# kkty/kmer-sets-compression

Hardware: AMD Instinct MI355X
Metric: Mk-mers/s processed in kmerset-multiple-compress; bytes/k-mer after SPSS (higher is better)
Workload: dtype u32

## Files before the change

### kmer-sets-compression_amd/csrc/ksh_encode.hip

```cpp
#include "ksh_internal.h"
#include "ksh_dsu.h"
#include "ksh_kmer.h"

#include <algorithm>
#include <cstddef>
#include <cstdlib>
#include <string>

namespace ksh {

#ifndef KSH_RULER_SHIFT
#define KSH_RULER_SHIFT 5
#endif
constexpr int kRulerShift = KSH_RULER_SHIFT;
constexpr uint32_t kRulerEvery = 1u << kRulerShift;

constexpr uint32_t kNone = 0xFFFFFFFFu;
constexpr uint32_t kMulti = 0xFFFFFFFEu;

#ifndef KSH_JUMP_HOPS
#define KSH_JUMP_HOPS 4
#endif
constexpr int kJumpHops = KSH_JUMP_HOPS;

#ifdef KSH_TRACE
__device__ unsigned long long* g_probe_trace = nullptr;
__device__ long long g_probe_trace_rows = 0;
#define KSH_PMARK(which, m)                                                                              \
  do {                                                                                                   \
    if (g_probe_trace && threadIdx.x == 0 && int64_t(blockIdx.x) < g_probe_trace_rows)                    \
      g_probe_trace[((which) * g_probe_trace_rows + blockIdx.x) * 16 + (m)] = __builtin_amdgcn_s_memtime(); \
  } while (0)
#define KSH_PMARK_WAVE(which)                                                                            \
  do {                                                                                                   \
    if (g_probe_trace && threadIdx.x % 64 == 0 && threadIdx.x / 64 < 16 && int64_t(blockIdx.x) < g_probe_trace_rows) \
      g_probe_trace[((which) * g_probe_trace_rows + blockIdx.x) * 16 + threadIdx.x / 64] = __builtin_amdgcn_s_memtime(); \
  } while (0)
#else
#define KSH_PMARK(which, m) do { } while (0)
#define KSH_PMARK_WAVE(which) do { } while (0)
#endif

template <typename KeyT>
__global__ __launch_bounds__(256) void k_fine_index(const int64_t* __restrict__ off,
                                                     const KeyT* __restrict__ keys, int key_bits,
                                                     int fine_bits, uint32_t* __restrict__ fine,
                                                     int64_t n_buckets) {
  extern __shared__ uint32_t s_fine[];
  const int64_t b = blockIdx.x;
  const int64_t lo = off[b], hi = off[b + 1];
  const int kSlices = 1 << fine_bits;
  const int sh = key_bits - fine_bits;
  uint32_t* f = fine + (b << fine_bits);
  if (lo == hi) {
    for (int sub = threadIdx.x; sub < kSlices; sub += 256) f[sub] = uint32_t(lo);
  } else {
    constexpr int kAhead = 4;
    for (int64_t base = lo; base < hi; base += 256 * kAhead) {
      KeyT cur_key[kAhead], prev_key[kAhead];
#pragma unroll
      for (int u = 0; u < kAhead; u++) {
        const int64_t i = base + u * 256 + threadIdx.x;
        if (i < hi) {
          cur_key[u] = keys[i];
          prev_key[u] = i > lo ? keys[i - 1] : KeyT(0);
        }
      }
#pragma unroll
      for (int u = 0; u < kAhead; u++) {
        const int64_t i = base + u * 256 + threadIdx.x;
        if (i < hi) {
          const int cur = int(uint64_t(cur_key[u]) >> sh);
          const int prev = i > lo ? int(uint64_t(prev_key[u]) >> sh) : -1;
          for (int sub = prev + 1; sub <= cur; sub++) s_fine[sub] = uint32_t(i);
        }
      }
    }
    const int last = int(uint64_t(keys[hi - 1]) >> sh);
    for (int sub = last + 1 + int(threadIdx.x); sub < kSlices; sub += 256) s_fine[sub] = uint32_t(hi);
    __syncthreads();
    for (int sub = threadIdx.x; sub < kSlices; sub += 256) f[sub] = s_fine[sub];
  }
  if (b == n_buckets - 1 && threadIdx.x == 0) fine[n_buckets << fine_bits] = uint32_t(hi);
}

template <typename KeyT>
__global__ __launch_bounds__(256) void k_coarse_index(DevSet<KeyT> set, int64_t n_entries, uint32_t* __restrict__ coarse) {
  const int64_t e = int64_t(blockIdx.x) * blockDim.x + threadIdx.x;
  if (e >= n_entries) return;
  const int64_t t = e << kCoarseShift;
  coarse[e] = uint32_t(set.bucket_search(t < set.n ? t : set.n - 1));
}

template <typename KeyT, bool kDirected, typename F>
__device__ __forceinline__ void for_side_neighbours(const DevSet<KeyT>& set, uint64_t x, uint64_t rx,
                                                    int64_t t, int side, F f) {
  const int k = set.k;
  if (kDirected) {
    if (side) {
      set.for_group4(kmer_next(x, k, 0), [&](int64_t idx) {
        if (idx != t) f(idx, 0u);
      });
    } else {
#pragma unroll
      for (int c = 0; c < 4; c++) {
        const uint64_t z = kmer_prev(x, k, c);
        if (z == x) continue;
        const int64_t idx = set.find(z);
        if (idx >= 0) f(idx, 0u);
      }
    }
    return;
  }
  set.for_group4(kmer_next(side ? x : rx, k, 0), [&](int64_t idx) {
    if (idx != t) f(idx, side ? 0u : 1u);
  });
  const uint64_t base = side ? rx : x;
#pragma unroll
  for (int c = 0; c < 4; c++) {
    const uint64_t z = kmer_prev(base, k, c);
    if (revcomp(z, k) < z) continue;
    if (z == x) continue;
    const int64_t idx = set.find(z);
    if (idx >= 0) f(idx, side ? 1u : 0u);
  }
}

template <typename KeyT, bool kDirected>
__global__ __launch_bounds__(256) void k_adjacency(DevSet<KeyT> set, uint32_t* __restrict__ nbr,
                                                    int* __restrict__ self_rc) {
  __shared__ int64_t s_bucket[2];
  const int64_t t = int64_t(blockIdx.x) * blockDim.x + threadIdx.x;
  const uint64_t x = set.kmer_in_block(t, s_bucket);
  if (t >= set.n) return;
  const uint64_t rx = kDirected ? 0 : revcomp(x, set.k);
  if (!kDirected && rx == x) *self_rc = 1;
  int cnt[2] = {0, 0};
  uint32_t single[2] = {kNone, kNone};
#pragma unroll
  for (int side = 0; side < 2; side++)
    for_side_neighbours<KeyT, kDirected>(set, x, rx, t, side, [&](int64_t idx, uint32_t same) {
      cnt[side]++;
      single[side] = (uint32_t(idx) << 1) | same;
    });
  nbr[2 * t] = cnt[0] == 0 ? kNone : (cnt[0] == 1 ? single[0] : kMulti);
  nbr[2 * t + 1] = cnt[1] == 0 ? kNone : (cnt[1] == 1 ? single[1] : kMulti);
}

template <typename KeyT, bool kDirected>
__global__ __launch_bounds__(256) void k_link_cut(DevSet<KeyT> set, uint32_t* __restrict__ nbr) {
  const int64_t t = int64_t(blockIdx.x) * blockDim.x + threadIdx.x;
  if (t >= set.n) return;
  const uint2 mine = reinterpret_cast<const uint2*>(nbr)[t];
  if (mine.x != kMulti && mine.y != kMulti) return;
  const uint64_t x = set.kmer(t);
  const uint64_t rx = kDirected ? 0 : revcomp(x, set.k);
  for (int side = 0; side < 2; side++) {
    if ((side ? mine.y : mine.x) != kMulti) continue;
    for_side_neighbours<KeyT, kDirected>(set, x, rx, t, side, [&](int64_t idx, uint32_t same) {
      uint32_t* facing = nbr + 2 * idx + (same ? side : side ^ 1);
      if (*reinterpret_cast<volatile uint32_t*>(facing) < kMulti) *reinterpret_cast<volatile uint32_t*>(facing) = kNone;
    });
    nbr[2 * t + side] = kNone;
  }
}

template <typename KeyT>
struct __attribute__((aligned(8))) RcRecord {
  KeyT key;
  uint32_t t;
};

template <typename KeyT>
__global__ __launch_bounds__(1024) void k_rc_hist(const KeyT* __restrict__ keys, int64_t n, int k, int key_bits,
                                                   int nbits, int64_t per_row,
                                                   uint32_t* __restrict__ hist_matrix) {
  extern __shared__ uint32_t lds_hist[];
  const int nb = 1 << nbits;
  for (int b = threadIdx.x; b < nb; b += blockDim.x) lds_hist[b] = 0u;
  __syncthreads();
  const int64_t t_begin = int64_t(blockIdx.x) * per_row;
  const int64_t t_end = min(t_begin + per_row, n);
  const int low_bits = 2 * k - 2 - nbits;
  for (int64_t t = t_begin + threadIdx.x; t < t_end; t += blockDim.x) {
    const uint64_t rx = revcomp(uint64_t(keys[t]), k);
    atomicAdd(&lds_hist[uint32_t(rx >> low_bits) & uint32_t(nb - 1)], 1u);
  }
  __syncthreads();
  uint32_t* my_row = hist_matrix + int64_t(blockIdx.x) * nb;
  for (int b = threadIdx.x; b < nb; b += blockDim.x) my_row[b] = lds_hist[b];
}

constexpr int kColTeams = 16;
__global__ __launch_bounds__(64 * kColTeams) void k_rc_columns(uint32_t* __restrict__ hist_matrix, int64_t n_rows,
                                                                int nb, int64_t* __restrict__ totals) {
  __shared__ uint32_t team_total[kColTeams][64];
  const int lane = threadIdx.x & 63, team = threadIdx.x >> 6;
  const int b = blockIdx.x * 64 + lane;
  const int64_t per_team = (n_rows + kColTeams - 1) / kColTeams;
  const int64_t g0 = min(int64_t(team) * per_team, n_rows), g1 = min(g0 + per_team, n_rows);
  uint32_t run = 0;
  if (b < nb)
    for (int64_t g = g0; g < g1; g++) run += hist_matrix[g * nb + b];
  team_total[team][lane] = run;
  __syncthreads();
  if (b >= nb) return;
  uint32_t before = 0, all = 0;
#pragma unroll
  for (int t2 = 0; t2 < kColTeams; t2++) {
    const uint32_t v = team_total[t2][lane];
    if (t2 < team) before += v;
    all += v;
  }
  run = before;
  for (int64_t g = g0; g < g1; g++) {
    uint32_t* cell = hist_matrix + g * nb + b;
    const uint32_t c = *cell;
    *cell = run;
    run += c;
  }
  if (team == 0) totals[b] = all;
}

template <typename KeyT>
__global__ __launch_bounds__(1024) void k_rc_scatter(DevSet<KeyT> set, int nbits, int round_bits, int round,
                                                      int64_t per_row,
                                                      const uint32_t* __restrict__ hist_matrix,
                                                      const int64_t* __restrict__ goff,
                                                      RcRecord<KeyT>* __restrict__ rec) {
  extern __shared__ uint32_t lds_hist[];
  const int nb = 1 << nbits;
  const uint32_t* my_row = hist_matrix + int64_t(blockIdx.x) * nb;
  for (int b = threadIdx.x; b < nb; b += blockDim.x) lds_hist[b] = uint32_t(goff[b]) + my_row[b];
  const int64_t t_begin = int64_t(blockIdx.x) * per_row;
  const int64_t t_end = min(t_begin + per_row, set.n);
  __syncthreads();
  if (t_begin >= t_end) return;
  const int64_t b_first = set.bucket_of(t_begin), b_last = set.bucket_of(t_end - 1);
  const int k = set.k, low_bits = 2 * set.k - 2 - nbits;
  const uint64_t low_mask = (uint64_t(1) << low_bits) - 1;
  for (int64_t t = t_begin + threadIdx.x; t < t_end; t += blockDim.x) {
    const uint64_t key = uint64_t(set.keys[t]);
    const uint32_t grp = uint32_t(revcomp(key, k) >> low_bits) & uint32_t(nb - 1);
    if (int(grp >> (nbits - round_bits)) != round) continue;
    int64_t lo = b_first, hi = b_last;
    while (lo < hi) {
      const int64_t mid = (lo + hi + 1) >> 1;
      if (set.off[mid] <= t) lo = mid; else hi = mid - 1;
    }
    const uint64_t rx = revcomp((uint64_t(lo) << set.key_bits) | key, k);
    const uint32_t dst = atomicAdd(&lds_hist[grp], 1u);
    RcRecord<KeyT> r;
    r.key = KeyT(((rx >> (2 * k - 2)) << low_bits) | (rx & low_mask));
    r.t = uint32_t(t);
    rec[dst] = r;
  }
}

constexpr int kSgBits = 7;
constexpr int kL1Threads = 1024;
constexpr int kL2Threads = 256;
constexpr int kL2Per = 8;
constexpr int kL2Tile = kL2Threads * kL2Per;

template <typename KeyT, int kPer>
__global__ __launch_bounds__(kL1Threads) void k_rc_scatter_l1(DevSet<KeyT> set, int nbits, int64_t per_row,
                                                               const uint32_t* __restrict__ hist_matrix,
                                                               const int64_t* __restrict__ goff,
                                                               RcRecord<KeyT>* __restrict__ tmp_rec,
                                                               uint16_t* __restrict__ tmp_g) {
  constexpr int kTile = kL1Threads * kPer;
  constexpr int kSg = 1 << kSgBits;
  __shared__ RcRecord<KeyT> s_rec[kTile];
  __shared__ uint16_t s_g[kTile];
  __shared__ uint32_t s_cur[kSg], s_cnt[kSg], s_lbase[kSg + 1];
  constexpr int kOffCap = 1024;
  __shared__ int64_t s_off[kOffCap];
  const int tid = threadIdx.x;
  const int nb = 1 << nbits, lo_bits = nbits - kSgBits;
  const uint32_t* my_row = hist_matrix + int64_t(blockIdx.x) * nb;
  if (tid < kSg) {
    uint32_t at = uint32_t(goff[int64_t(tid) << lo_bits]);
    for (int gi = 0; gi < (1 << lo_bits); gi++) at += my_row[(tid << lo_bits) + gi];
    s_cur[tid] = at;
    s_cnt[tid] = 0;
  }
  const int64_t t_begin = int64_t(blockIdx.x) * per_row;
  const int64_t t_end = min(t_begin + per_row, set.n);
  __syncthreads();
  if (t_begin >= t_end) return;
  const int64_t b_first = set.bucket_of(t_begin), b_last = set.bucket_of(t_end - 1);
  const int k = set.k, low_bits = 2 * set.k - 2 - nbits;
  const uint64_t low_mask = (uint64_t(1) << low_bits) - 1;
  const int n_span = int(min<int64_t>(b_last - b_first + 1, kOffCap + 1));
  const bool off_staged = n_span <= kOffCap;
  if (off_staged)
    for (int j = tid; j < n_span; j += kL1Threads) s_off[j] = set.off[b_first + j];
  __syncthreads();
  for (int64_t t0 = t_begin; t0 < t_end; t0 += kTile) {
    const int tile_n = int(min<int64_t>(kTile, t_end - t0));
    RcRecord<KeyT> mine[kPer];
    uint32_t grp[kPer], rank[kPer];
#pragma unroll
    for (int j = 0; j < kPer; j++) {
      const int64_t t = t0 + tid + j * kL1Threads;
      grp[j] = 0xFFFFFFFFu;
      if (t >= t_end) continue;
      const uint64_t key = uint64_t(set.keys[t]);
      int64_t lo = b_first, hi = b_last;
      if (off_staged) {
        int l2 = 0, h2 = n_span - 1;
        while (l2 < h2) {
          const int mid = (l2 + h2 + 1) >> 1;
          if (s_off[mid] <= t) l2 = mid; else h2 = mid - 1;
        }
        lo = b_first + l2;
// ... 483 lines not shown
      const int i = base + u * kThreads + tid;
      if (i < n_rec) chain_in(i, r[u]);
    }
  }
  __syncthreads();
  const auto walk = [&](uint32_t sl, auto f) {
    uint32_t j = head[sl];
    while (j != none) {
      if (kPacked) {
        const uint64_t e = entry[j];
        f(e & kf_mask, uint32_t(e >> t_shift));
        j = uint32_t(e >> kf_bits) & none;
      } else {
        const uint64_t key = uint64_t(rkey[j]);
        const uint32_t nj = nxt[j];
        f(((key >> (2 + e_sbits)) << 2) | (key & 3), rt[j]);
        j = uint32_t(nj);
      }
    }
  };
  const uint64_t hi_mask = (uint64_t(1) << (rest_bits - e_sbits)) - 1;
  const auto look0 = [&](int64_t i, KeyT ykey) {
    const uint64_t low = (uint64_t(ykey) >> 2) & low_mask;
    const uint64_t want = ((low >> (2 + e_sbits)) << 2) | (low & 3);
    int cnt = 0;
    uint32_t single = kNone;
    walk(uint32_t(low >> 2) & slice_mask, [&](uint64_t kf, uint32_t t) {
      if ((((kf >> 2) & hi_mask) << 2 | (kf & 3)) == want && t != uint32_t(i)) {
        cnt++;
        single = (t << 1) | 1u;
      }
    });
    return cnt == 0 ? kNone : (cnt == 1 ? single : kMulti);
  };
  const auto look1 = [&](int64_t i, int tb, KeyT key) {
    const uint64_t q = (uint64_t(tb) << rest_bits) | (uint64_t(key) & rest_mask);
    const uint64_t want = q >> e_sbits;
    int cnt = 0;
    uint32_t single = kNone;
    walk(uint32_t(q) & slice_mask, [&](uint64_t kf, uint32_t t) {
      if ((kf >> 2) == want && t != uint32_t(i)) {
        cnt++;
        single = (t << 1) | 1u;
      }
    });
    return cnt == 0 ? kNone : (cnt == 1 ? single : kMulti);
  };
  const auto merged = [](uint32_t now, uint32_t before) {
    const int total = (now == kNone ? 0 : (now == kMulti ? 2 : 1)) + (before == kNone ? 0 : (before == kMulti ? 2 : 1));
    return total == 0 ? kNone : (total > 1 ? kMulti : (now != kNone ? now : before));
  };
#pragma unroll 1
  for (int64_t i = p0_lo + tid; i < p0_hi; i += kThreads) {
    const KeyT ykey = y_next;
    if (i + kThreads < p0_hi) y_next = set.keys[i + kThreads];
    rc0[i] = look0(i, ykey);
  }
#pragma unroll 1
  for (int idx = tid; idx < total; idx += kThreads) {
    const int tb = tb_next;
    const int64_t i = i_next;
    const KeyT key = key_next;
    if (idx + kThreads < total) {
      i_next = place(idx + kThreads, &tb_next);
      key_next = set.keys[i_next];
    }
    rc1[i] = look1(i, tb, key);
  }
#pragma unroll 1
  for (int64_t rb = r0 + cap; rb < r1; rb += cap) {
    const int n_b = int(r1 - rb < int64_t(cap) ? r1 - rb : int64_t(cap));
    __syncthreads();
    for (int sl = tid; sl < n_slices; sl += kThreads) head[sl] = none;
    __syncthreads();
    for (int i = tid; i < n_b; i += kThreads) chain_in(i, rec[rb + i]);
    __syncthreads();
    for (int64_t i = p0_lo + tid; i < p0_hi; i += kThreads) {
      const uint32_t now = look0(i, set.keys[i]);
      if (now != kNone) rc0[i] = merged(now, rc0[i]);
    }
    for (int idx = tid; idx < total; idx += kThreads) {
      int tb;
      const int64_t i = place(idx, &tb);
      const uint32_t now = look1(i, tb, set.keys[i]);
      if (now != kNone) rc1[i] = merged(now, rc1[i]);
    }
  }
}

constexpr int kFwdChunk = 512;
template <typename KeyT>
struct FwdCfg {
  static constexpr int kCapNext = 3072;
  static constexpr int kCapPrev = 512;
  static_assert(kCapPrev % kFwdChunk == 0 && kCapNext % kFwdChunk == 0, "staging shape");
};
constexpr int kFwdSpan = 16;

constexpr int kFwdBounds = 12;

template <typename KeyT>
__global__ __launch_bounds__(256) void k_fwd_bounds(DevSet<KeyT> set, int64_t n_chunks,
                                                     int64_t* __restrict__ bounds) {
  const int64_t id = int64_t(blockIdx.x) * blockDim.x + threadIdx.x;
  const int64_t c = id / 10;
  const int j = int(id - c * 10);
  if (c > n_chunks) return;
  const int k = set.k;
  const int64_t t = c * kFwdChunk;
  int64_t* out = bounds + kFwdBounds * c;
  if (j < 5) {
    if (t < set.n) {
      const uint64_t x = set.kmer(t);
      out[j] = lower_bound_kmer(set, j == 0 ? kmer_next(x, k, 0) : kmer_prev(x, k, j - 1));
      if (j == 0) out[10] = int64_t(x);
    }
  } else if (t > 0) {
    const uint64_t y = set.kmer((t < set.n ? t : set.n) - 1);
    out[j] = lower_bound_kmer(set, (j == 5 ? kmer_next(y, k, 3) : kmer_prev(y, k, j - 6)) + 1);
    if (j == 5) out[11] = int64_t(y);
  }
}

template <typename KeyT>
__device__ __forceinline__ int lds_lower_bound(const KeyT* a, int lo, int hi, KeyT key) {
  int len = hi - lo;
  if (len <= 0) return lo;
  while (len > 1) {
    const int half = len >> 1;
    lo = a[lo + half - 1] < key ? lo + half : lo;
    len -= half;
  }
  return lo + (a[lo] < key ? 1 : 0);
}
template <typename KeyT>
__device__ __forceinline__ int lds_find(const KeyT* a, int lo, int hi, KeyT key) {
  int len = hi - lo;
  if (len <= 0) return -1;
  while (len > 1) {
    const int half = len >> 1;
    lo = a[lo + half - 1] < key ? lo + half : lo;
    len -= half;
  }
  const KeyT at = a[lo];
  if (at == key) return lo;
  return (at < key && lo + 1 < hi && a[lo + 1] == key) ? lo + 1 : -1;
}

__device__ unsigned long long g_fwd_dbg[8];


template <typename KeyT, int kFwdCapNext = FwdCfg<KeyT>::kCapNext>
__global__ __launch_bounds__(kFwdChunk, (sizeof(KeyT) <= 4 ? 8 : 4)) void k_adj_fwd_staged(DevSet<KeyT> set, const int64_t* __restrict__ bounds,
                                                              const uint32_t* __restrict__ rc0,
                                                              const uint32_t* __restrict__ rc1,
                                                              uint32_t* __restrict__ nbr,
                                                              int* __restrict__ self_rc) {
  constexpr int kFwdCapPrev = FwdCfg<KeyT>::kCapPrev;
  static_assert(kFwdCapNext % kFwdChunk == 0, "staging shape");
  __shared__ KeyT s_next[kFwdCapNext];
  __shared__ KeyT s_prev[4][kFwdCapPrev];
  __shared__ int64_t s_b[2 * kFwdBounds];
  __shared__ int s_rel[6][kFwdSpan + 1];
  const int tid = threadIdx.x;
  const int64_t chunk = blockIdx.x;
  const int64_t t = chunk * kFwdChunk + tid;
  const int k = set.k;
  KSH_PMARK(0, 0);
  if (tid < 2 * kFwdBounds) s_b[tid] = bounds[kFwdBounds * chunk + tid];
  KeyT my_key = 0;
  uint2 rc = make_uint2(kNone, kNone);
  if (t < set.n) {
    my_key = set.keys[t];
    rc = make_uint2(rc0[t], rc1[t]);
  }
  __syncthreads();
  KSH_PMARK(0, 1);
  const uint64_t x_first = uint64_t(s_b[10]), x_last = uint64_t(s_b[kFwdBounds + 11]);
  int fb[6];
  fb[0] = int(kmer_next(x_first, k, 0) >> set.key_bits);
#pragma unroll
  for (int cc = 0; cc < 4; cc++) fb[1 + cc] = int(kmer_prev(x_first, k, cc) >> set.key_bits);
  fb[5] = int(x_first >> set.key_bits);
  bool usable[5];
  int len[5];
  int64_t lo_of[5];
#pragma unroll
  for (int r = 0; r < 5; r++) {
    lo_of[r] = s_b[r];
    const int64_t l = s_b[kFwdBounds + 5 + r] - lo_of[r];
    usable[r] = l >= 0 && l <= (r == 0 ? kFwdCapNext : kFwdCapPrev);
    len[r] = usable[r] ? int(l) : 0;
  }
  if ((x_first >> (2 * k - 2)) != (x_last >> (2 * k - 2))) {
    usable[0] = false;
    len[0] = 0;
  }
  if (tid < 6 * (kFwdSpan + 1)) {
    const int r = tid / (kFwdSpan + 1), j = tid % (kFwdSpan + 1);
    const int64_t b = int64_t(fb[r]) + j;
    const int64_t at = b <= set.n_buckets ? set.off[b] : set.n;
    int64_t rel;
    if (r < 5) {
      int64_t lo_r = lo_of[0];
      int len_r = len[0];
#pragma unroll
      for (int q = 1; q < 5; q++)
        if (r == q) {
          lo_r = lo_of[q];
          len_r = len[q];
        }
      rel = at - lo_r;
      rel = rel < 0 ? 0 : (rel > len_r ? len_r : rel);
    } else {
      rel = at - chunk * kFwdChunk;
      rel = rel < -(int64_t(1) << 30) ? -(int64_t(1) << 30) : (rel > (int64_t(1) << 30) ? (int64_t(1) << 30) : rel);
    }
    s_rel[r][j] = int(rel);
  }
  {
    constexpr int kPer = kFwdCapNext / kFwdChunk, kPerPrev = kFwdCapPrev / kFwdChunk;
    KeyT vn[kPer], vp[4][kPerPrev];
#pragma unroll
    for (int u = 0; u < kPer; u++)
      if (tid + u * kFwdChunk < len[0]) vn[u] = set.keys[lo_of[0] + tid + u * kFwdChunk];
#pragma unroll
    for (int cc = 0; cc < 4; cc++)
#pragma unroll
      for (int u = 0; u < kPerPrev; u++)
        if (tid + u * kFwdChunk < len[1 + cc]) vp[cc][u] = set.keys[lo_of[1 + cc] + tid + u * kFwdChunk];
#pragma unroll
    for (int u = 0; u < kPer; u++)
      if (tid + u * kFwdChunk < len[0]) s_next[tid + u * kFwdChunk] = vn[u];
#pragma unroll
    for (int cc = 0; cc < 4; cc++)
#pragma unroll
      for (int u = 0; u < kPerPrev; u++)
        if (tid + u * kFwdChunk < len[1 + cc]) s_prev[cc][tid + u * kFwdChunk] = vp[cc][u];
    KSH_PMARK(0, 2);
  }
  __syncthreads();
  KSH_PMARK(0, 3);
  if (t >= set.n) return;
  int64_t my_b = fb[5];
  {
    int j = 0;
    while (j < kFwdSpan && s_rel[5][j + 1] <= tid) j++;
    my_b += j;
    if (j == kFwdSpan)
      while (set.off[my_b + 1] <= t) my_b++;
  }
  const uint64_t x = (uint64_t(my_b) << set.key_bits) | uint64_t(my_key);
  const uint64_t rx = revcomp(x, k);
  const uint64_t rx_next = (rx << 2) & kmer_mask(k);
  if (rx == x) *self_rc = 1;
  int cnt[2] = {0, 0};
  uint32_t single[2] = {kNone, kNone};
  const auto bucket_range = [&](int r, int b, int* lo, int* hi) {
    const int j = b - fb[r];
    if (j < 0 || j >= kFwdSpan) return false;
    *lo = s_rel[r][j];
    *hi = s_rel[r][j + 1];
    return true;
  };
  const uint32_t t32 = uint32_t(t);
  uint32_t lo32[5];
#pragma unroll
  for (int r = 0; r < 5; r++) lo32[r] = uint32_t(lo_of[r]);
  uint32_t pend = 0;
  const uint64_t g0 = kmer_next(x, k, 0);
  {
    int lo, hi;
#ifdef KSH_FWD_DEBUG
    atomicAdd(&g_fwd_dbg[0], 1ull);
    if (!usable[0]) atomicAdd(&g_fwd_dbg[1], 1ull);
    else if (!bucket_range(0, int(g0 >> set.key_bits), &lo, &hi)) atomicAdd(&g_fwd_dbg[2], 1ull);
    if (s_b[kFwdBounds + 5] - s_b[0] > kFwdCapNext) atomicAdd(&g_fwd_dbg[5], 1ull);
    if ((x_first >> (2 * k - 2)) != (x_last >> (2 * k - 2))) atomicAdd(&g_fwd_dbg[6], 1ull);
#endif
    if (usable[0] && bucket_range(0, int(g0 >> set.key_bits), &lo, &hi)) {
      const KeyT gkey = KeyT(g0 & set.key_mask());
      if (lo < hi) {
        int i = lds_lower_bound(s_next, lo, hi, gkey);
        for (; i < hi && KeyT(s_next[i] - gkey) < KeyT(4); i++) {
          const uint32_t idx = lo32[0] + uint32_t(i);
          if (idx == t32) continue;
          cnt[1]++;
          single[1] = idx << 1;
        }
      }
    } else {
      pend |= 16u;
    }
  }
  KSH_PMARK(0, 4);
#pragma unroll
  for (int c = 0; c < 4; c++) {
    const uint64_t z = kmer_prev(x, k, c);
    if ((rx_next | uint64_t(3 - c)) < z) continue;
    if (z == x) continue;
    int lo, hi;
#ifdef KSH_FWD_DEBUG
    if (!usable[1 + c]) atomicAdd(&g_fwd_dbg[3], 1ull);
    else if (!bucket_range(1 + c, int(z >> set.key_bits), &lo, &hi)) atomicAdd(&g_fwd_dbg[4], 1ull);
#endif
    if (usable[1 + c] && bucket_range(1 + c, int(z >> set.key_bits), &lo, &hi)) {
      const KeyT zkey = KeyT(z & set.key_mask());
      const int i = lds_find(s_prev[c], lo, hi, zkey);
      if (i >= 0) {
        cnt[0]++;
        single[0] = (lo32[1 + c] + uint32_t(i)) << 1;
      }
    } else {
      pend |= 1u << c;
    }
  }
  if (pend & 16u)
    set.for_group4(g0, [&](int64_t idx) {
      if (idx == t) return;
      cnt[1]++;
      single[1] = uint32_t(idx) << 1;
    });
  pend &= 15u;
#pragma unroll 1
  while (pend) {
    const int c = __ffs(int(pend)) - 1;
    pend &= pend - 1;
    const int64_t idx = set.find(kmer_prev(x, k, c));
    if (idx >= 0) {
      cnt[0]++;
      single[0] = uint32_t(idx) << 1;
    }
  }
  KSH_PMARK(0, 5);
  const uint32_t r[2] = {rc.x, rc.y};
  uint32_t out[2];
#pragma unroll
  for (int side = 0; side < 2; side++) {
    const int total = cnt[side] + (r[side] == kNone ? 0 : (r[side] == kMulti ? 2 : 1));
    out[side] = total == 0 ? kNone : (total > 1 ? kMulti : (cnt[side] == 1 ? single[side] : r[side]));
  }
  reinterpret_cast<uint2*>(nbr)[t] = make_uint2(out[0], out[1]);
  KSH_PMARK(0, 6);
}

#ifndef KSH_TGT_CHUNK
#define KSH_TGT_CHUNK 2048
#endif
#ifndef KSH_TGT_CHUNK64
#define KSH_TGT_CHUNK64 2048
#endif
template <typename KeyT>
struct TgtCfg {
  static constexpr int kChunk = sizeof(KeyT) == 8 ? KSH_TGT_CHUNK64 : KSH_TGT_CHUNK;
  static constexpr int kStreamMax = 2 * kChunk;
};
#ifndef KSH_TGT_THREADS
#define KSH_TGT_THREADS 512
#endif
constexpr int kTgtThreads = KSH_TGT_THREADS;
constexpr int kTgtSpan = 16;
constexpr int kTgtBounds = 6;
struct TgtTask {
  int64_t c;
  int j, m;
};

template <typename KeyT>
__global__ __launch_bounds__(256) void k_tgt_bounds(DevSet<KeyT> set, int64_t n_chunks, int64_t* __restrict__ bounds) {
  const int64_t id = int64_t(blockIdx.x) * blockDim.x + threadIdx.x;
  const int64_t c = id >> 3;
  const int j = int(id & 7);
  const bool live = c <= n_chunks;
  const int k = set.k;
  const int64_t base = (live ? c : 0) * TgtCfg<KeyT>::kChunk;
  const int64_t p = base - 1 + j;
  uint64_t pref = ~uint64_t(0);
  if (live && j < 5 && p >= 0 && p < set.n) pref = set.kmer(p) >> 2;
  const int lane0 = int(threadIdx.x & 63) & ~7;
  const uint64_t before = __shfl(pref, lane0, 64);
  const bool breaks = j >= 1 && j < 5 && (p >= set.n || pref != before);
  const unsigned long long m = __ballot(breaks) >> lane0;
  const int first = __ffsll((long long)(m & 0x1Eull)) - 1;
  int64_t b = base - 1 + first;
  uint64_t v = __shfl(pref, lane0 + (first > 0 ? first : 0), 64);
  if (c == 0) {
    b = 0;
    v = 0;
  } else if (b >= set.n) {
    b = set.n;
    v = uint64_t(1) << (2 * k - 2);
  }
  if (!live) return;
  if (j < 4) bounds[kTgtBounds * c + 2 + j] = lower_bound_kmer(set, (uint64_t(j) << (2 * k - 2)) + v);
  if (j == 4) {
    bounds[kTgtBounds * c] = b;
    bounds[kTgtBounds * c + 1] = int64_t(v);
  }
}

__global__ __launch_bounds__(256) void k_tgt_split(const int64_t* __restrict__ cuts, int64_t n_chunks, int64_t cap,
                                                    int stream_max, int64_t* __restrict__ rec,
                                                    TgtTask* __restrict__ task, int* __restrict__ n_extra) {
  const int64_t c = int64_t(blockIdx.x) * blockDim.x + threadIdx.x;
  if (c >= n_chunks) return;
  const int64_t* lo = cuts + kTgtBounds * c;
  const int64_t* hi = lo + kTgtBounds;
  int64_t stream = 0;
#pragma unroll
  for (int a = 0; a < 4; a++) stream += hi[2 + a] - lo[2 + a];
  int64_t* r = rec + 2 * kTgtBounds * c;
#pragma unroll
  for (int i = 0; i < kTgtBounds; i++) r[i] = lo[i];
  const int64_t m = (stream + stream_max - 1) / stream_max;
  int64_t e = 0;
  if (m > 1) {
    e = int64_t(atomicAdd(n_extra, int(m - 1)));
    if (e + m - 1 > cap) {
      atomicSub(n_extra, int(m - 1));
      e = -1;
    }
  }
  if (m <= 1 || e < 0) {
#pragma unroll
    for (int i = 0; i < kTgtBounds; i++) r[kTgtBounds + i] = hi[i];
    return;
  }
  for (int64_t j = 1; j < m; j++) task[e + j - 1] = TgtTask{c, int(j), int(m)};
}

template <typename KeyT>
__global__ __launch_bounds__(256) void k_tgt_subcuts(DevSet<KeyT> set, const int64_t* __restrict__ cuts, int64_t n_chunks,
                                                      int64_t cap, const TgtTask* __restrict__ task,
                                                      const int* __restrict__ n_extra, int64_t* __restrict__ rec) {
  const int64_t id = int64_t(blockIdx.x) * blockDim.x + threadIdx.x;
  const int64_t e = id >> 3;
  const int lane = int(id & 7);
  const int64_t count = *n_extra < cap ? int64_t(*n_extra) : cap;
  if (e >= count || lane > 4) return;
  const TgtTask t = task[e];
  const int k = set.k;
  const int64_t* lo_c = cuts + kTgtBounds * t.c;
  const int64_t* hi_c = lo_c + kTgtBounds;
  int best = 0;
  int64_t best_len = hi_c[2] - lo_c[2];
#pragma unroll
  for (int a = 1; a < 4; a++) {
    const int64_t len = hi_c[2 + a] - lo_c[2 + a];
    if (len > best_len) {
      best_len = len;
      best = a;
    }
  }
  const int64_t pos = lo_c[2 + best] + int64_t((uint64_t(best_len) * uint64_t(t.j)) / uint64_t(t.m));
  const uint64_t v = set.kmer(pos) & ((uint64_t(1) << (2 * k - 2)) - 1);
  const int64_t at = lane < 4 ? lower_bound_kmer(set, (uint64_t(lane) << (2 * k - 2)) + v) : lower_bound_kmer(set, v << 2);
  const int slot = lane < 4 ? 2 + lane : 0;
  int64_t* mine = rec + 2 * kTgtBounds * (n_chunks + e);
  int64_t* before = rec + 2 * kTgtBounds * (t.j == 1 ? t.c : n_chunks + e - 1) + kTgtBounds;
  mine[slot] = at;
  before[slot] = at;
  if (lane == 4) {
    mine[1] = int64_t(v);
    before[1] = int64_t(v);
  }
  if (t.j == t.m - 1) {
    const int64_t* hi = cuts + kTgtBounds * (t.c + 1);
    mine[kTgtBounds + slot] = hi[slot];
    if (lane == 4) mine[kTgtBounds + 1] = hi[1];
  }
}

__device__ __forceinline__ uint32_t side_verdict(uint32_t direct, uint32_t through_rc) {
  const int total = (direct == kNone ? 0 : (direct == kMulti ? 2 : 1)) + (through_rc == kNone ? 0 : (through_rc == kMulti ? 2 : 1));
  return total == 0 ? kNone : (total > 1 ? kMulti : (direct != kNone ? direct : through_rc));
}

template <typename KeyT>
__global__ __launch_bounds__(kTgtThreads, 8) void k_adj_fwd_targets(DevSet<KeyT> set, const int64_t* __restrict__ rec,
                                                                   int64_t n_chunks, const int* __restrict__ n_extra,
                                                                   const uint32_t* __restrict__ rc0,
                                                                   const uint32_t* __restrict__ rc1,
                                                                   uint32_t* __restrict__ nbr, int* __restrict__ self_rc) {
  constexpr int kRounds = (TgtCfg<KeyT>::kChunk + 3 + kTgtThreads - 1) / kTgtThreads;
  __shared__ KeyT s_keys[kRounds * kTgtThreads];
  __shared__ uint32_t s_slot[kRounds * kTgtThreads];
  __shared__ int64_t s_b[2 * kTgtBounds];
  __shared__ int s_rel[5 * (kTgtSpan + 1)];
  const int tid = threadIdx.x;
  const int64_t chunk = blockIdx.x;
  const int k = set.k;
  KSH_PMARK(0, 0);
  if (chunk >= n_chunks && chunk - n_chunks >= int64_t(*n_extra)) return;
  if (tid < 2 * kTgtBounds) s_b[tid] = rec[2 * kTgtBounds * chunk + tid];
  __syncthreads();
  KSH_PMARK(0, 1);
  const int64_t b = s_b[0];
  const int len_w = int(s_b[kTgtBounds] - b);
  const uint64_t v = uint64_t(s_b[1]);
  const auto first_bucket = [&](int r) {
    return int((r == 4 ? (v << 2) : ((uint64_t(r) << (2 * k - 2)) | v)) >> set.key_bits);
  };
  const int fb_w = first_bucket(4);
  if (tid < 5 * (kTgtSpan + 1)) {
    const int r = tid / (kTgtSpan + 1), j = tid % (kTgtSpan + 1);
    const int64_t bb = int64_t(first_bucket(r)) + j;
    const int64_t at = bb <= set.n_buckets ? set.off[bb] : set.n;
    const int64_t lo_r = r == 4 ? b : s_b[2 + r];
    const int64_t len_r = r == 4 ? int64_t(len_w) : s_b[kTgtBounds + 2 + r] - lo_r;
    int64_t rel = at - lo_r;
    rel = rel < 0 ? 0 : (rel > len_r ? len_r : rel);
    s_rel[r * (kTgtSpan + 1) + j] = int(rel);
  }
  KeyT wk[kRounds];
  uint32_t wr[kRounds];
#pragma unroll
  for (int u = 0; u < kRounds; u++) {
    const int i = tid + u * kTgtThreads;
    wr[u] = kNone;
    if (i < len_w) {
      wk[u] = set.keys[b + i];
      wr[u] = rc0[b + i];
    }
  }
#pragma unroll
  for (int u = 0; u < kRounds; u++) {
    const int i = tid + u * kTgtThreads;
    if (i < len_w) s_keys[i] = wk[u];
    s_slot[i] = wr[u];
  }
  KSH_PMARK(0, 2);
  __shared__ uint32_t s_qbase[4];
  __shared__ int s_cum[4], s_fb[4];
  const int c1 = int(s_b[kTgtBounds + 2] - s_b[2]), c2 = c1 + int(s_b[kTgtBounds + 3] - s_b[3]),
            c3 = c2 + int(s_b[kTgtBounds + 4] - s_b[4]);
  const int total = c3 + int(s_b[kTgtBounds + 5] - s_b[5]);
  if (tid < 4) {
    const int cum = tid == 0 ? 0 : (tid == 1 ? c1 : (tid == 2 ? c2 : c3));
    s_cum[tid] = cum;
    s_qbase[tid] = uint32_t(s_b[2 + tid]) - uint32_t(cum);
    s_fb[tid] = first_bucket(tid);
  }
  const uint32_t b32 = uint32_t(b);
  const bool even_k = (k & 1) == 0;
  __syncthreads();
  KSH_PMARK(0, 3);
  const auto range_of = [&](int idx) { return (idx >= c1 ? 1 : 0) + (idx >= c2 ? 1 : 0) + (idx >= c3 ? 1 : 0); };
  KeyT key_next = 0;
  uint32_t rc_next = kNone;
  if (tid < total) {
    const uint32_t p = s_qbase[range_of(tid)] + uint32_t(tid);
    key_next = set.keys[p];
    rc_next = rc1[p];
  }
#pragma unroll 1
  for (int idx = tid; idx < total; idx += kTgtThreads) {
    const int a = range_of(idx);
    const int r = idx - s_cum[a];
    const uint32_t p32 = s_qbase[a] + uint32_t(idx);
    const KeyT key = key_next;
    const uint32_t through_rc = rc_next;
    if (idx + kTgtThreads < total) {
      const uint32_t p2 = s_qbase[range_of(idx + kTgtThreads)] + uint32_t(idx + kTgtThreads);
      key_next = set.keys[p2];
      rc_next = rc1[p2];
    }
    int64_t my_b;
    {
      const int row = a * (kTgtSpan + 1);
      int j = 0;
      while (j < kTgtSpan && s_rel[row + j + 1] <= r) j++;
      my_b = j < kTgtSpan ? int64_t(s_fb[a] + j) : set.bucket_of(int64_t(p32));
    }
    const uint64_t x = (uint64_t(my_b) << set.key_bits) | uint64_t(key);
    if (even_k && revcomp(x, k) == x) *self_rc = 1;
    const uint64_t g0 = kmer_next(x, k, 0);
    int cnt = 0;
    uint32_t single = kNone;
    const int jw = int(g0 >> set.key_bits) - fb_w;
    if (jw >= 0 && jw < kTgtSpan) {
      const int lo = s_rel[4 * (kTgtSpan + 1) + jw], hi = s_rel[4 * (kTgtSpan + 1) + jw + 1];
      const KeyT gkey = KeyT(g0 & set.key_mask());
      if (lo < hi) {
        int i = lds_lower_bound(s_keys, lo, hi, gkey);
        for (; i < hi && KeyT(s_keys[i] - gkey) < KeyT(4); i++) {
          const uint32_t at = b32 + uint32_t(i);
          if (at == p32) continue;
          cnt++;
          single = at << 1;
          mark_hit(&s_slot[i], p32 << 1);
        }
      }
    } else {
      set.for_group4(g0, [&](int64_t at) {
        if (uint32_t(at) == p32) return;
        cnt++;
        single = uint32_t(at) << 1;
        const int64_t i = at - b;
        if (i >= 0 && i < len_w) mark_hit(&s_slot[i], p32 << 1);
      });
    }
    const uint32_t direct = cnt == 0 ? kNone : (cnt == 1 ? single : kMulti);
    nbr[2 * size_t(p32) + 1] = side_verdict(direct, through_rc);
  }
  KSH_PMARK(0, 4);
  __syncthreads();
  KSH_PMARK(0, 5);
#pragma unroll
  for (int u = 0; u < kRounds; u++) {
    const int i = tid + u * kTgtThreads;
    if (i < len_w) nbr[2 * (b + i)] = s_slot[i];
  }
  KSH_PMARK(0, 6);
#ifdef KSH_TRACE
  if (g_probe_trace && tid == 0 && chunk < g_probe_trace_rows) g_probe_trace[chunk * 16 + 7] = (unsigned long long)(total);
#endif
}

template <typename KeyT>
__global__ __launch_bounds__(256) void k_adj_fwd(DevSet<KeyT> set, const uint32_t* __restrict__ rc0,
                                                  const uint32_t* __restrict__ rc1,
                                                  uint32_t* __restrict__ nbr, int* __restrict__ self_rc) {
  __shared__ int64_t s_bucket[2];
  const int64_t t = int64_t(blockIdx.x) * blockDim.x + threadIdx.x;
  const uint64_t x = set.kmer_in_block(t, s_bucket);
  if (t >= set.n) return;
  const int k = set.k;
  if (revcomp(x, k) == x) *self_rc = 1;
  int cnt[2] = {0, 0};
  uint32_t single[2] = {kNone, kNone};
  set.for_group4(kmer_next(x, k, 0), [&](int64_t idx) {
    if (idx == t) return;
    cnt[1]++;
    single[1] = uint32_t(idx) << 1;
  });
#pragma unroll
  for (int c = 0; c < 4; c++) {
    const uint64_t z = kmer_prev(x, k, c);
    if (revcomp(z, k) < z) continue;
    if (z == x) continue;
    const int64_t idx = set.find(z);
    if (idx < 0) continue;
    cnt[0]++;
    single[0] = uint32_t(idx) << 1;
  }
  const uint32_t r[2] = {rc0[t], rc1[t]};
  uint32_t out[2];
#pragma unroll
  for (int side = 0; side < 2; side++) {
    const int total = cnt[side] + (r[side] == kNone ? 0 : (r[side] == kMulti ? 2 : 1));
    out[side] = total == 0 ? kNone : (total > 1 ? kMulti : (cnt[side] == 1 ? single[side] : r[side]));
  }
  reinterpret_cast<uint2*>(nbr)[t] = make_uint2(out[0], out[1]);
}

__device__ __forceinline__ uint2 link_pair(const uint32_t* __restrict__ link, uint32_t s) {
  return reinterpret_cast<const uint2*>(link)[s >> 1];
}
__device__ __forceinline__ uint32_t leave_link(uint2 pr, uint32_t s) { return (s & 1) ? pr.x : pr.y; }
__device__ __forceinline__ uint32_t enter_link(uint2 pr, uint32_t s) { return (s & 1) ? pr.y : pr.x; }
__device__ __forceinline__ uint32_t step_to(uint32_t s, uint32_t lk) {
  return ((lk >> 1) << 1) | ((s & 1) ^ (lk & 1));
}

__device__ __forceinline__ bool sampled_ruler(uint32_t s) { return (s & (2u * kRulerEvery - 2u)) == 0; }

constexpr uint64_t kRecUnset = ~uint64_t(0);
constexpr uint64_t kEndFlag = uint64_t(1) << 63;

__device__ __forceinline__ uint32_t dense_index(uint32_t s) { return ((s >> (kRulerShift + 1)) << 1) | (s & 1); }
__device__ __forceinline__ uint64_t make_rec(uint32_t kind, uint32_t off, uint32_t ref) {
  return (uint64_t(kind) << 62) | (uint64_t(off & 0x3FFFFFFFu) << 32) | ref;
}
__device__ __forceinline__ uint64_t make_rinfo(bool end, uint32_t dist, uint32_t nx) {
  return (end ? kEndFlag : 0) | (uint64_t(dist & 0x7FFFFFFFu) << 32) | nx;
}

__global__ __launch_bounds__(256) void k_ruler_walk(const uint32_t* __restrict__ link,
                                                     int64_t n_states, int64_t n_dense,
                                                     unsigned long long* __restrict__ rinfo,
                                                     unsigned long long* __restrict__ rec) {
  const int64_t i = int64_t(blockIdx.x) * blockDim.x + threadIdx.x;
  if (i >= n_dense) return;
  const int64_t s64 = 2 * int64_t(kRulerEvery) * (i >> 1) + (i & 1);
  if (s64 >= n_states) {
    rinfo[i] = make_rinfo(true, 0, 0);
    return;
  }
  const uint32_t r = uint32_t(s64);
  uint32_t lk = leave_link(link_pair(link, r), r);
  if ((r & 1) == 0) rec[r] = make_rec(0, 0, uint32_t(i));
  if (lk == kNone) {
    rinfo[i] = make_rinfo(true, 0, r);
    return;
  }
  uint32_t cur = r, steps = 0;
  while (true) {
    cur = step_to(cur, lk);
    steps++;
    if (sampled_ruler(cur) || steps >= 0x3FFFFFFFu) {
      rinfo[i] = make_rinfo(false, steps, cur);
      return;
    }
    if ((cur & 1) == 0) rec[cur] = make_rec(0, steps, uint32_t(i));
    lk = leave_link(link_pair(link, cur), cur);
    if (lk == kNone) {
      rinfo[i] = make_rinfo(true, steps, cur);
      return;
    }
  }
}

__device__ __forceinline__ uint64_t make_chain_info(bool ruler_ahead, uint32_t steps, uint32_t ref) {
  return (ruler_ahead ? kEndFlag : 0) | (uint64_t(steps & 0x7FFFFFFFu) << 32) | ref;
}

__global__ __launch_bounds__(256) void k_ruler_heads(const uint32_t* __restrict__ link,
                                                      const uint32_t* __restrict__ ends, int64_t n_ends,
                                                      unsigned long long* __restrict__ rec,
                                                      unsigned long long* __restrict__ chain_info) {
  const int64_t e = int64_t(blockIdx.x) * blockDim.x + threadIdx.x;
  if (e >= n_ends) return;
  const int64_t t = ends[e];
  if ((t & (kRulerEvery - 1)) == 0) return;
  const uint2 own = reinterpret_cast<const uint2*>(link)[t];
  const uint32_t flags = (own.x == kNone ? 1u : 0u) | (own.y == kNone ? 2u : 0u);
  if (!flags) return;
  for (uint32_t d = 0; d < 2; d++) {
    if (!(flags & (1u << d))) continue;
    const uint32_t s0 = uint32_t(2 * t) | d;
    uint32_t lk = leave_link(link_pair(link, s0), s0);
    if (lk == kNone) {
      rec[s0] = make_rec(2, 0, s0);
      continue;
    }
    uint32_t cur = s0, off = 0;
    while (true) {
      if ((cur & 1) == 0) rec[cur] = make_rec(3, off, s0);
      cur = step_to(cur, lk);
      off++;
      if (sampled_ruler(cur)) {
        chain_info[t] = make_chain_info(true, off, dense_index(cur));
        break;
      }
      lk = leave_link(link_pair(link, cur), cur);
      if (lk == kNone || off >= 0x3FFFFFFFu) {
        if ((cur & 1) == 0) rec[cur] = make_rec(3, off, s0);
        chain_info[t] = make_chain_info(false, off, cur);
        break;
      }
    }
  }
}

__device__ __forceinline__ unsigned long long rec_look(const unsigned long long* p) {
  return __hip_atomic_load(p, __ATOMIC_RELAXED, __HIP_MEMORY_SCOPE_AGENT);
}
__device__ __forceinline__ void rec_post(unsigned long long* p, unsigned long long v) {
  __hip_atomic_store(p, v, __ATOMIC_RELAXED, __HIP_MEMORY_SCOPE_AGENT);
}
__device__ __forceinline__ bool first_phase(uint32_t s) {
  return (((s >> 1) * 0x9E3779B1u) >> 13 ^ s) & 1u;
}

struct WalkLog {
  unsigned long long* hdr;
  uint32_t* mid;
  int64_t n_walkers;
  int n_mid;
  int k;
  uint32_t* long_walkers;
  unsigned int* long_count;
  uint32_t long_tag;
  __device__ __forceinline__ bool is_long(uint32_t steps) const { return steps > uint32_t(n_mid + 1) * uint32_t(k); }
  __device__ __forceinline__ void arrived(int64_t w, uint32_t steps, uint32_t state) const {
    if (!hdr) return;
    hdr[w] = (uint64_t(steps) << 32) | state;
    if (is_long(steps)) long_walkers[atomicAdd(long_count, 1u)] = uint32_t(w) | long_tag;
  }
  __device__ __forceinline__ void passed(int64_t w, int j, uint32_t state) const {
    if (hdr && j < n_mid) mid[int64_t(j) * n_walkers + w] = state;
  }
};
constexpr int kLogMidRulers = 7, kLogMidHeads = 7;

template <int kPhase>
__global__ __launch_bounds__(256) void k_rank_walk(const uint32_t* __restrict__ link, int64_t n_states,
                                                    int64_t n_dense, unsigned long long* __restrict__ rinfo,
                                                    unsigned long long* __restrict__ chain_info, WalkLog log,
                                                    unsigned long long* __restrict__ unset_a,
                                                    unsigned long long* __restrict__ unset_b) {
  const int64_t i = int64_t(blockIdx.x) * blockDim.x + threadIdx.x;
  if (i >= n_dense) return;
  if (unset_a) {
    unset_a[i] = ~0ull;
    unset_b[i] = ~0ull;
  }
  const int64_t s64 = 2 * int64_t(kRulerEvery) * (i >> 1) + (i & 1);
  if (s64 >= n_states) {
    rinfo[i] = make_rinfo(true, 0, 0);
    return;
  }
  const uint32_t r = uint32_t(s64);
  if (kPhase == 1 && !first_phase(r)) return;
  if (rec_look(rinfo + i) != kRecUnset) return;
  const uint2 own = link_pair(link, r);
  uint32_t lk = leave_link(own, r);
  if (lk == kNone) {
    rec_post(rinfo + i, make_rinfo(true, 0, r));
    if (enter_link(own, r) == kNone) log.arrived(i, 0, r);
    return;
  }
  uint32_t cur = r, steps = 0;
  int since = 0, n_passed = 0;
  while (true) {
    cur = step_to(cur, lk);
    steps++;
    if (sampled_ruler(cur) || steps >= 0x3FFFFFFFu) {
      rec_post(rinfo + i, make_rinfo(false, steps, cur));
      rec_post(rinfo + dense_index(cur ^ 1), make_rinfo(false, steps, r ^ 1));
      log.arrived(i, steps, cur);
      return;
    }
    if (++since == log.k) {
      since = 0;
      log.passed(i, n_passed++, cur);
    }
    lk = leave_link(link_pair(link, cur), cur);
    if (lk == kNone) {
      rec_post(rinfo + i, make_rinfo(true, steps, cur));
      rec_post(chain_info + (cur >> 1), make_chain_info(true, steps, dense_index(r ^ 1)));
      log.arrived(i, steps, cur);
      return;
    }
  }
}

template <int kPhase>
__global__ __launch_bounds__(256) void k_rank_heads(const uint32_t* __restrict__ link,
                                                     const uint32_t* __restrict__ ends, int64_t n_ends,
                                                     unsigned long long* __restrict__ rinfo,
                                                     unsigned long long* __restrict__ chain_info, WalkLog log) {
  const int64_t e = int64_t(blockIdx.x) * blockDim.x + threadIdx.x;
  if (e >= n_ends) return;
  const uint32_t t = ends[e];
  if ((t & (kRulerEvery - 1)) == 0) return;
  const uint2 own = reinterpret_cast<const uint2*>(link)[t];
  uint32_t s0;
  if (own.x == kNone && own.y != kNone) {
    s0 = 2 * t;
  } else if (own.y == kNone && own.x != kNone) {
    s0 = 2 * t + 1;
  } else {
    log.arrived(e, 0, 2 * t);
    return;
  }
  if (kPhase == 1 && !first_phase(s0)) return;
  if (rec_look(chain_info + t) != kRecUnset) return;
  uint32_t lk = leave_link(own, s0);
  uint32_t cur = s0, off = 0;
  int since = 0, n_passed = 0;
  while (true) {
    cur = step_to(cur, lk);
    off++;
    if (sampled_ruler(cur)) {
      rec_post(chain_info + t, make_chain_info(true, off, dense_index(cur)));
      rec_post(rinfo + dense_index(cur ^ 1), make_rinfo(true, off, s0 ^ 1));
      log.arrived(e, off, cur);
      return;
    }
    if (++since == log.k) {
      since = 0;
      log.passed(e, n_passed++, cur);
    }
    lk = leave_link(link_pair(link, cur), cur);
    if (lk == kNone || off >= 0x3FFFFFFFu) {
      rec_post(chain_info + t, make_chain_info(false, off, cur));
      rec_post(chain_info + (cur >> 1), make_chain_info(false, off, s0 ^ 1));
      log.arrived(e, off, cur);
      return;
    }
  }
}

__global__ __launch_bounds__(256) void k_rank_unset(const uint32_t* __restrict__ ends, int64_t n_ends,
                                                     unsigned long long* __restrict__ chain_info) {
  const int64_t e = int64_t(blockIdx.x) * blockDim.x + threadIdx.x;
  if (e < n_ends) chain_info[ends[e]] = kRecUnset;
}

__global__ __launch_bounds__(256) void k_ruler_jump(int64_t n_dense,
                                                     unsigned long long* __restrict__ rinfo,
                                                     const int* __restrict__ prev,
                                                     int* __restrict__ changed) {
  if (prev && *prev == 0) return;
  const int64_t i = int64_t(blockIdx.x) * blockDim.x + threadIdx.x;
  if (i >= n_dense) return;
  uint64_t mine = rinfo[i];
  if (mine & kEndFlag) return;
#pragma unroll
  for (int hop = 0; hop < kJumpHops && !(mine & kEndFlag); hop++) {
    const uint64_t theirs = rinfo[dense_index(uint32_t(mine))];
    const uint32_t dist = uint32_t((mine >> 32) & 0x7FFFFFFFu) + uint32_t((theirs >> 32) & 0x7FFFFFFFu);
    mine = (theirs & kEndFlag) | (uint64_t(dist & 0x7FFFFFFFu) << 32) | uint32_t(theirs);
  }
  rinfo[i] = mine;
  *changed = 1;
}

#ifndef KSH_L2_SHIFT
#define KSH_L2_SHIFT 4
#endif
constexpr int kL2Shift = KSH_L2_SHIFT;
__device__ __forceinline__ bool is_level2(int64_t i) { return ((i >> 1) & ((1 << kL2Shift) - 1)) == 0; }
__device__ __forceinline__ int64_t level2_index(int64_t i) { return ((i >> (kL2Shift + 1)) << 1) | (i & 1); }
__device__ __forceinline__ int64_t level2_entry(int64_t j) { return ((j >> 1) << (kL2Shift + 1)) | (j & 1); }

template <bool kLevel2>
__global__ __launch_bounds__(256) void k_l2_walk(const unsigned long long* __restrict__ rinfo, int64_t n_dense,
                                                  unsigned long long* __restrict__ r2,
                                                  unsigned long long* __restrict__ head,
                                                  unsigned long long* __restrict__ stamp) {
  const int64_t at = int64_t(blockIdx.x) * blockDim.x + threadIdx.x;
  const int64_t i = kLevel2 ? level2_entry(at) : at;
  if (i >= n_dense) return;
  const bool l2 = kLevel2;
  if (!kLevel2 && (is_level2(i) || !(rinfo[i ^ 1] & kEndFlag))) return;
  uint64_t dist = 0;
  int64_t cur = i;
  uint64_t out;
  for (int64_t steps = 0;; steps++) {
    const uint64_t ri = rinfo[cur];
    dist += (ri >> 32) & 0x7FFFFFFFu;
    if (ri & kEndFlag) {
      out = kEndFlag | ((dist & 0x7FFFFFFFu) << 32) | uint32_t(ri);
      break;
    }
    cur = dense_index(uint32_t(ri));
    if (is_level2(cur) || steps > n_dense) {
      out = ((dist & 0x7FFFFFFFu) << 32) | uint32_t(cur);
      break;
    }
    stamp[cur] = (dist << 32) | uint32_t(i);
  }
  if (l2) r2[level2_index(i)] = out; else head[i] = out;
}

__global__ __launch_bounds__(256) void k_l2_jump(int64_t n_l2, unsigned long long* __restrict__ r2,
                                                  const int* __restrict__ prev, int* __restrict__ changed) {
  if (prev && *prev == 0) return;
  const int64_t j = int64_t(blockIdx.x) * blockDim.x + threadIdx.x;
  if (j >= n_l2) return;
  uint64_t mine = r2[j];
  if (mine & kEndFlag) return;
#pragma unroll
  for (int hop = 0; hop < kJumpHops && !(mine & kEndFlag); hop++) {
    const uint64_t theirs = r2[level2_index(int64_t(uint32_t(mine)))];
    const uint32_t dist = uint32_t((mine >> 32) & 0x7FFFFFFFu) + uint32_t((theirs >> 32) & 0x7FFFFFFFu);
    mine = (theirs & kEndFlag) | (uint64_t(dist & 0x7FFFFFFFu) << 32) | uint32_t(theirs);
  }
  r2[j] = mine;
  *changed = 1;
}

__device__ __forceinline__ uint64_t l2_walker_end(int64_t w, const unsigned long long* __restrict__ r2,
                                                  const unsigned long long* __restrict__ head) {
  if (is_level2(w)) return r2[level2_index(w)];
  const uint64_t h = head[w];
  if (h & kEndFlag) return h;
  const uint64_t ahead = r2[level2_index(int64_t(uint32_t(h)))];
  const uint32_t dist = uint32_t((h >> 32) & 0x7FFFFFFFu) + uint32_t((ahead >> 32) & 0x7FFFFFFFu);
  return (ahead & kEndFlag) | (uint64_t(dist & 0x7FFFFFFFu) << 32) | uint32_t(ahead);
}

__global__ __launch_bounds__(256) void k_l2_resolve(int64_t n_dense, const unsigned long long* __restrict__ r2,
                                                     const unsigned long long* __restrict__ head,
                                                     const unsigned long long* __restrict__ stamp,
                                                     unsigned long long* __restrict__ rinfo) {
  const int64_t i = int64_t(blockIdx.x) * blockDim.x + threadIdx.x;
  if (i >= n_dense) return;
  const uint64_t mine = rinfo[i];
  if (mine & kEndFlag) return;
  if (is_level2(i) || head[i] != kRecUnset) {
    rinfo[i] = l2_walker_end(i, r2, head);
    return;
  }
  const uint64_t st = stamp[i];
  if (st == kRecUnset) return;
  const uint64_t we = l2_walker_end(int64_t(uint32_t(st)), r2, head);
  const uint32_t dist = uint32_t((we >> 32) & 0x7FFFFFFFu) - uint32_t(st >> 32);
  rinfo[i] = (we & kEndFlag) | (uint64_t(dist & 0x7FFFFFFFu) << 32) | uint32_t(we);
}

__device__ __forceinline__ uint64_t mirror_rec(uint64_t r) { return r ^ ((uint64_t(1) << 62) | 1u); }

__device__ __forceinline__ bool resolve_rec(uint64_t r, const unsigned long long* __restrict__ rinfo,
                                            uint32_t* end, uint32_t* dist) {
  if (r == kRecUnset) return false;
  const uint32_t kind = uint32_t(r >> 62), off = uint32_t((r >> 32) & 0x3FFFFFFFu), ref = uint32_t(r);
  if (kind == 2) {
    *end = ref;
    *dist = off;
    return true;
  }
  const uint64_t ri = rinfo[ref];
  if (!(ri & kEndFlag)) return false;
  const uint32_t rd = uint32_t((ri >> 32) & 0x7FFFFFFFu);
  *end = uint32_t(ri);
  *dist = kind == 0 ? rd - off : rd + off;
  return true;
}

constexpr int kLenSums = 32;
struct Chosen {
  uint32_t head_state;
  uint32_t p;
  uint32_t len;
  uint32_t d;
  uint32_t last;
  uint8_t cls;
};
__device__ __forceinline__ Chosen choose_from_ends(uint32_t e0, uint32_t d0, uint32_t e1, uint32_t d1,
                                                   bool directed) {
  const uint32_t fwd_start = e1 >> 1, fwd_end = e0 >> 1;
  Chosen c;
  c.d = (directed || fwd_start >= fwd_end) ? 0u : 1u;
  c.head_state = (c.d ? e0 : e1) ^ 1;
  c.p = c.d ? d0 : d1;
  c.len = d0 + d1 + 1;
  c.last = c.d ? e1 : e0;
  c.cls = (directed || fwd_start == fwd_end) ? uint8_t(0) : uint8_t((c.head_state & 1) == 0 ? 1 : 2);
  return c;
}

__device__ __forceinline__ uint8_t ori_byte(uint32_t d, uint32_t to_far_end) {
  return uint8_t((d & 1u) | ((to_far_end & 15u) << 1));
}

__global__ __launch_bounds__(256) void k_choose(const unsigned long long* __restrict__ rec,
                                                 const unsigned long long* __restrict__ rinfo,
                                                 const unsigned long long* __restrict__ chain_info,
                                                 int64_t n, bool directed, uint32_t* __restrict__ head,
                                                 uint32_t* __restrict__ pos,
                                                 uint8_t* __restrict__ ori,
                                                 uint8_t* __restrict__ hcls,
                                                 uint32_t* __restrict__ hlen,
                                                 uint32_t* __restrict__ hlast) {
  const int64_t t = int64_t(blockIdx.x) * blockDim.x + threadIdx.x;
  if (t >= n) return;
  ulonglong2 both = reinterpret_cast<const ulonglong2*>(rec)[t];
  uint32_t e0, d0, e1, d1;
  bool ok;
  if (both.x != kRecUnset && (both.x >> 62) == 3) {
    const uint32_t off = uint32_t((both.x >> 32) & 0x3FFFFFFFu), start = uint32_t(both.x);
    const uint64_t ci = chain_info[start >> 1];
    const uint32_t steps = uint32_t((ci >> 32) & 0x7FFFFFFFu);
    ok = true;
    if (ci & kEndFlag) {
      const uint64_t ri = rinfo[uint32_t(ci)];
      ok = (ri & kEndFlag) != 0;
      e0 = uint32_t(ri);
      d0 = steps - off + uint32_t((ri >> 32) & 0x7FFFFFFFu);
    } else {
      e0 = uint32_t(ci);
      d0 = steps - off;
    }
    e1 = start ^ 1;
    d1 = off;
  } else {
    if (both.y == kRecUnset && both.x != kRecUnset && (both.x >> 62) < 2) both.y = mirror_rec(both.x);
    ok = resolve_rec(both.x, rinfo, &e0, &d0) && resolve_rec(both.y, rinfo, &e1, &d1);
  }
  if (!ok) {
    head[t] = kNone;
    hcls[t] = 0xFE;
    return;
  }
  const Chosen c = choose_from_ends(e0, d0, e1, d1, directed);
  head[t] = c.head_state >> 1;
  pos[t] = c.p;
  ori[t] = ori_byte(c.d, c.len - 1 - c.p);
  hcls[t] = c.p == 0 ? c.cls : uint8_t(0xFF);
  if (c.p == 0) {
    hlen[t] = c.len;
    hlast[t] = c.last;
  }
}

__device__ __forceinline__ bool chain_end_of(uint32_t s, uint2 own, const unsigned long long* __restrict__ rinfo,
                                             const unsigned long long* __restrict__ chain_info,
                                             uint32_t* end, uint32_t* dist) {
  if (leave_link(own, s) == kNone) {
    *end = s;
    *dist = 0;
    return true;
  }
  if (sampled_ruler(s)) {
    const uint64_t ri = rinfo[dense_index(s)];
    *end = uint32_t(ri);
    *dist = uint32_t((ri >> 32) & 0x7FFFFFFFu);
    return (ri & kEndFlag) != 0;
  }
  const uint64_t ci = chain_info[s >> 1];
  const uint32_t steps = uint32_t((ci >> 32) & 0x7FFFFFFFu);
  if (!(ci & kEndFlag)) {
    *end = uint32_t(ci);
    *dist = steps;
    return true;
  }
  const uint64_t ri = rinfo[uint32_t(ci)];
  *end = uint32_t(ri);
  *dist = steps + uint32_t((ri >> 32) & 0x7FFFFFFFu);
  return (ri & kEndFlag) != 0;
}

__device__ __forceinline__ bool choose_at(uint32_t t, uint2 own, const unsigned long long* __restrict__ rinfo,
                                          const unsigned long long* __restrict__ chain_info, bool directed,
                                          Chosen* c) {
  uint32_t e0, d0, e1, d1;
  const bool ok0 = chain_end_of(2 * t, own, rinfo, chain_info, &e0, &d0);
  const bool ok1 = chain_end_of(2 * t + 1, own, rinfo, chain_info, &e1, &d1);
  if (!(ok0 && ok1)) return false;
  *c = choose_from_ends(e0, d0, e1, d1, directed);
  return true;
}

__global__ __launch_bounds__(256) void k_choose_ends(const uint32_t* __restrict__ link,
                                                      const uint32_t* __restrict__ ends, int64_t n_ends,
                                                      const unsigned long long* __restrict__ rinfo,
                                                      const unsigned long long* __restrict__ chain_info,
                                                      bool directed, uint32_t* __restrict__ head,
                                                      uint8_t* __restrict__ ori, uint8_t* __restrict__ hcls,
                                                      uint32_t* __restrict__ hlen, uint32_t* __restrict__ hlast,
                                                      unsigned long long* __restrict__ len_sums,
                                                      int* __restrict__ loop_flag) {
  __shared__ unsigned long long s_len;
  if (threadIdx.x == 0) s_len = 0;
  __syncthreads();
  const int64_t e = int64_t(blockIdx.x) * blockDim.x + threadIdx.x;
  if (e < n_ends) {
    const uint32_t t = ends[e];
    const uint2 own = reinterpret_cast<const uint2*>(link)[t];
    Chosen c;
    if (!choose_at(t, own, rinfo, chain_info, directed, &c)) {
      *loop_flag = 1;
    } else {
      head[t] = c.head_state >> 1;
      if (c.p == 0) {
        hcls[t] = c.cls;
        hlen[t] = c.len;
        hlast[t] = c.last;
        ori[t] = uint8_t(c.d);
        atomicAdd(&s_len, static_cast<unsigned long long>(c.len));
      }
    }
  }
  __syncthreads();
  if (threadIdx.x == 0 && s_len) atomicAdd(len_sums + (blockIdx.x & (kLenSums - 1)), s_len);
}

__global__ __launch_bounds__(256) void k_rulers_done(const unsigned long long* __restrict__ rinfo, int64_t n_dense,
                                                      int* __restrict__ loop_flag) {
  const int64_t i = int64_t(blockIdx.x) * blockDim.x + threadIdx.x;
  if (i < n_dense && !(rinfo[i] & kEndFlag)) *loop_flag = 1;
}

__global__ __launch_bounds__(256) void k_loops(const uint32_t* __restrict__ link,
                                                int64_t n, uint32_t* __restrict__ head,
                                                uint32_t* __restrict__ pos,
                                                uint8_t* __restrict__ ori,
                                                uint8_t* __restrict__ hcls,
                                                uint32_t* __restrict__ hlen,
                                                uint32_t* __restrict__ hlast) {
  const int64_t t = int64_t(blockIdx.x) * blockDim.x + threadIdx.x;
  if (t >= n) return;
  if (hcls[t] != 0xFE) return;
  const uint32_t start = uint32_t(2 * t);
  uint32_t s = start;
  int64_t steps = 0;
  do {
    const uint32_t lk = link[s ^ 1];
    if (lk == kNone) return;
    s = ((lk >> 1) << 1) | ((s & 1) ^ (lk & 1));
    if ((s >> 1) < uint32_t(t)) return;
    steps++;
  } while (s != start && steps <= 2 * n);
  if (s != start) return;
  const uint32_t len = uint32_t(steps);
  uint32_t p = 0, last = start;
  s = start;
  do {
    const uint32_t y = s >> 1;
    head[y] = uint32_t(t);
    pos[y] = p;
    ori[y] = ori_byte(s & 1, len - 1 - p);
    last = s;
    const uint32_t lk = link[s ^ 1];
    s = ((lk >> 1) << 1) | ((s & 1) ^ (lk & 1));
    p++;
  } while (s != start);
  hcls[t] = 3;
  hlen[t] = p;
  hlast[t] = last;
}

constexpr int kHeadItems = 8;
constexpr int kHeadSpan = 256 * kHeadItems;

__device__ __forceinline__ uint64_t head_counts8(const uint8_t* __restrict__ hcls, int64_t t0, int64_t n,
                                                 uint8_t (&c)[kHeadItems]) {
  uint64_t packed = 0;
  if (t0 + kHeadItems <= n) {
    const uint2 v = *reinterpret_cast<const uint2*>(hcls + t0);
#pragma unroll
    for (int i = 0; i < kHeadItems; i++) c[i] = uint8_t(((i < 4 ? v.x : v.y) >> (8 * (i & 3))) & 0xFF);
  } else {
#pragma unroll
    for (int i = 0; i < kHeadItems; i++) c[i] = t0 + i < n ? hcls[t0 + i] : uint8_t(0xFF);
  }
#pragma unroll
  for (int i = 0; i < kHeadItems; i++)
    if (c[i] <= 3) packed += uint64_t(1) << (16 * c[i]);
  return packed;
}

__device__ __forceinline__ uint64_t block_scan_packed(uint64_t v, uint64_t* lds4, uint64_t* total) {
  const int lane = threadIdx.x & 63, wave = threadIdx.x >> 6;
  uint64_t inc = v;
#pragma unroll
  for (int d = 1; d < 64; d <<= 1) {
    const uint64_t o = __shfl_up(inc, d, 64);
    if (lane >= d) inc += o;
  }
  if (lane == 63) lds4[wave] = inc;
  __syncthreads();
  uint64_t before = 0;
#pragma unroll
  for (int w = 0; w < 4; w++)
    if (w < wave) before += lds4[w];
  *total = lds4[0] + lds4[1] + lds4[2] + lds4[3];
  return before + inc;
}

__device__ __forceinline__ uint32_t end_flags8(const uint32_t* __restrict__ link, int64_t t0, int64_t n) {
  uint32_t flags = 0;
#pragma unroll
  for (int i = 0; i < kHeadItems; i += 2) {
    if (t0 + i + 1 < n) {
      const uint4 v = *reinterpret_cast<const uint4*>(link + 2 * (t0 + i));
      if (v.x == kNone || v.y == kNone) flags |= 1u << i;
      if (v.z == kNone || v.w == kNone) flags |= 1u << (i + 1);
    } else if (t0 + i < n) {
      const uint2 v = *reinterpret_cast<const uint2*>(link + 2 * (t0 + i));
      if (v.x == kNone || v.y == kNone) flags |= 1u << i;
    }
  }
  return flags;
}

__global__ __launch_bounds__(256) void k_end_counts(const uint32_t* __restrict__ link, int64_t n,
                                                     int64_t* __restrict__ counts, uint8_t* __restrict__ flags8) {
  __shared__ uint64_t lds4[4];
  const int64_t t0 = (int64_t(blockIdx.x) * 256 + threadIdx.x) * kHeadItems;
  const uint32_t flags = end_flags8(link, t0, n);
  flags8[int64_t(blockIdx.x) * 256 + threadIdx.x] = uint8_t(flags);
  uint64_t total;
  (void)block_scan_packed(uint64_t(__popc(flags)), lds4, &total);
  if (threadIdx.x == 0) counts[blockIdx.x] = int64_t(total);
}

__global__ __launch_bounds__(256) void k_end_fill(const uint8_t* __restrict__ flags8, int64_t n,
                                                   const int64_t* __restrict__ before,
                                                   uint32_t* __restrict__ ends, uint8_t* __restrict__ hcls) {
  __shared__ uint64_t lds4[4];
  const int64_t t0 = (int64_t(blockIdx.x) * 256 + threadIdx.x) * kHeadItems;
  static_assert(kHeadItems == 8, "one 8-byte store per thread");
  if (t0 + kHeadItems <= n) {
    *reinterpret_cast<uint64_t*>(hcls + t0) = ~uint64_t(0);
  } else {
    for (int64_t t = t0; t < n; t++) hcls[t] = 0xFF;
  }
  const uint32_t flags = flags8[int64_t(blockIdx.x) * 256 + threadIdx.x];
  const uint64_t mine = uint64_t(__popc(flags));
  uint64_t total;
  int64_t at = before[blockIdx.x] + int64_t(block_scan_packed(mine, lds4, &total) - mine);
#pragma unroll
  for (int i = 0; i < kHeadItems; i++)
    if (flags & (1u << i)) ends[at++] = uint32_t(t0 + i);
}

__global__ __launch_bounds__(256) void k_head_block_counts(const uint8_t* __restrict__ hcls, int64_t n,
                                                            int64_t* __restrict__ b01,
                                                            int64_t* __restrict__ b23) {
  __shared__ uint64_t lds4[4];
  const int64_t t0 = (int64_t(blockIdx.x) * 256 + threadIdx.x) * kHeadItems;
  uint8_t c[kHeadItems];
  uint64_t total;
  (void)block_scan_packed(head_counts8(hcls, t0, n, c), lds4, &total);
  if (threadIdx.x == 0) {
    b01[blockIdx.x] = int64_t(total & 0xFFFF) | (int64_t((total >> 16) & 0xFFFF) << 32);
    b23[blockIdx.x] = int64_t((total >> 32) & 0xFFFF) | (int64_t(total >> 48) << 32);
  }
}

__global__ __launch_bounds__(256) void k_unitig_fill(
    const uint8_t* __restrict__ hcls, const int64_t* __restrict__ b01,
    const int64_t* __restrict__ b23, int64_t n, int64_t base1, int64_t base2, int64_t base3,
    const uint8_t* __restrict__ ori, const uint32_t* __restrict__ hlen,
    const uint32_t* __restrict__ hlast, uint32_t* __restrict__ uid, uint32_t* __restrict__ u_head,
    uint32_t* __restrict__ u_first, uint32_t* __restrict__ u_last, uint32_t* __restrict__ u_len) {
  __shared__ uint64_t lds4[4];
  const int64_t t0 = (int64_t(blockIdx.x) * 256 + threadIdx.x) * kHeadItems;
  uint8_t c[kHeadItems];
  const uint64_t mine = head_counts8(hcls, t0, n, c);
  uint64_t total;
  const uint64_t excl = block_scan_packed(mine, lds4, &total) - mine;
  if (mine == 0) return;
  const int64_t w01 = b01[blockIdx.x], w23 = b23[blockIdx.x];
  int64_t next[4] = {(w01 & 0xFFFFFFFF) + int64_t(excl & 0xFFFF),
                     base1 + (w01 >> 32) + int64_t((excl >> 16) & 0xFFFF),
                     base2 + (w23 & 0xFFFFFFFF) + int64_t((excl >> 32) & 0xFFFF),
                     base3 + (w23 >> 32) + int64_t(excl >> 48)};
#pragma unroll
  for (int i = 0; i < kHeadItems; i++) {
    if (c[i] > 3) continue;
    const int64_t t = t0 + i;
    const int64_t u = c[i] == 0 ? next[0]++ : c[i] == 1 ? next[1]++ : c[i] == 2 ? next[2]++ : next[3]++;
    uid[t] = uint32_t(u);
    u_head[u] = uint32_t(t);
    u_first[u] = uint32_t(2 * t) | (ori[t] & 1u);
    u_last[u] = hlast[t];
    u_len[u] = hlen[t];
  }
}

template <typename KeyT>
__global__ __launch_bounds__(256) void k_edges(DevSet<KeyT> set, int64_t n_vertices, bool directed,
                                                const uint32_t* __restrict__ u_first,
                                                const uint32_t* __restrict__ u_last,
                                                const uint32_t* __restrict__ head,
                                                const uint32_t* __restrict__ uid,
                                                uint32_t* __restrict__ edges, uint32_t* __restrict__ mate) {
  const int64_t v = int64_t(blockIdx.x) * blockDim.x + threadIdx.x;
  if (v >= n_vertices) return;
  mate[v] = kNone;
  const uint32_t u = uint32_t(v >> 1), side = uint32_t(v & 1);
  const uint32_t st = side ? u_last[u] : u_first[u];
  const int k = set.k;
  const uint64_t x = set.kmer(st >> 1);
  const uint64_t o = (st & 1) ? revcomp(x, k) : x;
  uint32_t out[4] = {kNone, kNone, kNone, kNone};
  const auto take = [&](int c, int64_t i, bool as_is) {
    const uint32_t u2 = uid[head[i]];
    if (u2 == u) return;
    if (directed) {
      out[c] = 2 * u2 + (side ? 0u : 1u);
      return;
    }
    const uint32_t f = side ? (as_is ? 0u : 1u) : (as_is ? 1u : 0u);
    const uint32_t fs = u_first[u2];
    const uint32_t side2 = ((fs >> 1) == uint32_t(i) && (fs & 1) == f) ? 0u : 1u;
    out[c] = 2 * u2 + side2;
  };
  if (side) {
    set.for_group4(kmer_next(o, k, 0), [&](int64_t i) { take(set.last_base(i), i, true); });
    if (!directed) {
#pragma unroll
      for (int c = 0; c < 4; c++) {
        const uint64_t y = kmer_next(o, k, c), r = revcomp(y, k);
        if (r < y) {
          const int64_t i = set.find(r);
          if (i >= 0) take(c, i, false);
        }
      }
    }
  } else {
#pragma unroll
    for (int c = 0; c < 4; c++) {
      const uint64_t y = kmer_prev(o, k, c);
      if (directed || y <= revcomp(y, k)) {
        const int64_t i = set.find(y);
        if (i >= 0) take(c, i, true);
      }
    }
    if (!directed) {
      const uint64_t ro = revcomp(o, k);
      set.for_group4(kmer_next(ro, k, 0), [&](int64_t i) {
        const int c = 3 - set.last_base(i);
        const uint64_t y = kmer_prev(o, k, c);
        if (revcomp(y, k) < y) take(c, i, false);
      });
    }
  }
  *reinterpret_cast<uint4*>(edges + 4 * v) = make_uint4(out[0], out[1], out[2], out[3]);
}

__device__ __forceinline__ uint64_t slot_priority(uint32_t v, int c, bool directed) {
  if (directed && !(v & 1)) return ~uint64_t(0);
  return uint64_t(v >> 1) * 8 + ((v & 1) ? 0 : 4) + uint64_t(c);
}

__global__ __launch_bounds__(256) void k_match_best(const uint32_t* __restrict__ edges,
                                                     const uint32_t* __restrict__ mate,
                                                     int64_t n_vertices, bool directed,
                                                     unsigned long long* __restrict__ best_prio,
                                                     uint32_t* __restrict__ best_w,
                                                     const int* __restrict__ prev,
                                                     int* __restrict__ any_live) {
  if (prev && *prev == 0) return;
  const int64_t v = int64_t(blockIdx.x) * blockDim.x + threadIdx.x;
  if (v >= n_vertices) return;
  uint32_t bw = kNone;
  uint64_t bp = ~uint64_t(0);
// ... 282 lines not shown
    bool one_sequence, int k, uint32_t* __restrict__ sid_at, uint32_t* __restrict__ lens,
    int64_t* __restrict__ str_bases) {
  const int64_t u = int64_t(blockIdx.x) * blockDim.x + threadIdx.x;
  if (u >= n_u) return;
  const int64_t base1 = class_totals[0] & 0xFFFFFFFF, base2 = base1 + (class_totals[0] >> 32);
  const uint8_t c = scls[u];
  if (c == 0xFF) return;
  int64_t sid;
  if (one_sequence || c == 0) sid = c01[u] & 0xFFFFFFFF;
  else if (c == 1) sid = base1 + (c01[u] >> 32);
  else sid = base2 + c2[u];
  sid_at[u] = uint32_t(sid);
  lens[sid] = uint32_t(s_nk[u] - 1);
  str_bases[sid] = s_nk[u] + k - 1;
}

__global__ __launch_bounds__(256) void k_string_assign(
    const uint32_t* __restrict__ u_len, const unsigned long long* __restrict__ walk, int64_t n_u,
    const uint8_t* __restrict__ scls, const uint32_t* __restrict__ sid_at, bool one_sequence,
    uint32_t* __restrict__ u_sid, uint32_t* __restrict__ u_koff, uint8_t* __restrict__ u_flip,
    const int* __restrict__ unfinished) {
  if (unfinished && *unfinished) return;
  const int64_t u = int64_t(blockIdx.x) * blockDim.x + threadIdx.x;
  if (u >= n_u) return;
  const unsigned long long wr = walk[2 * u + 1], wl = walk[2 * u];
  const uint32_t e_r = walk_next(wr) >> 1, e_l = walk_next(wl) >> 1;
  if (e_r == uint32_t(u) && e_l == uint32_t(u)) {
    u_sid[u] = sid_at[u];
    u_koff[u] = 0;
    u_flip[u] = (scls[u] == 2 && one_sequence) ? 1 : 0;
    return;
  }
  const bool from_left = scls[e_l] != 0xFF;
  const uint32_t start = from_left ? e_l : e_r;
  u_sid[u] = sid_at[start];
  u_koff[u] = (from_left ? walk_weight(wl) : walk_weight(wr)) - u_len[u];
  u_flip[u] = from_left ? 0 : 1;
}

__global__ __launch_bounds__(256) void k_unitig_strings(const uint32_t* __restrict__ u_len,
                                                         int64_t n_u, int k,
                                                         uint32_t* __restrict__ u_sid,
                                                         uint32_t* __restrict__ u_koff,
                                                         uint8_t* __restrict__ u_flip,
                                                         uint32_t* __restrict__ lens,
                                                         int64_t* __restrict__ str_bases) {
  const int64_t u = int64_t(blockIdx.x) * blockDim.x + threadIdx.x;
  if (u >= n_u) return;
  u_sid[u] = uint32_t(u);
  u_koff[u] = 0;
  u_flip[u] = 0;
  lens[u] = u_len[u] - 1;
  str_bases[u] = int64_t(u_len[u]) + k - 1;
}

struct UnitigPlace {
  int64_t base;
  uint32_t len;
  uint32_t flags;
};

__global__ __launch_bounds__(256) void k_unitig_place(const uint32_t* __restrict__ u_len,
                                                       const uint32_t* __restrict__ u_sid,
                                                       const uint32_t* __restrict__ u_koff,
                                                       const uint8_t* __restrict__ u_flip,
                                                       const int64_t* __restrict__ str_start,
                                                       const uint32_t* __restrict__ lens,
                                                       const uint32_t* __restrict__ u_head, int64_t n_u,
                                                       UnitigPlace* __restrict__ place_at_head,
                                                       const int* __restrict__ unfinished) {
  if (unfinished && *unfinished) return;
  const int64_t u = int64_t(blockIdx.x) * blockDim.x + threadIdx.x;
  if (u >= n_u) return;
  const uint32_t sid = u_sid[u];
  UnitigPlace pl;
  pl.base = str_start[sid] + u_koff[u];
  pl.len = u_len[u];
  const bool is_last = u_koff[u] + u_len[u] == lens[sid] + 1;
  pl.flags = uint32_t(u_flip[u] & 1) | (is_last ? 2u : 0u);
  place_at_head[u_head[u]] = pl;
}

template <int kEmitBases>
__device__ __forceinline__ void store_bases(uint8_t* __restrict__ at, uint64_t o, int k, bool writer, bool tail) {
  if (writer) {
    if (kEmitBases == 1) {
      at[0] = uint8_t((o >> (2 * (k - 1))) & 3);
    } else {
      struct __attribute__((packed, aligned(1))) Run {
        uint32_t w[kEmitBases / 4];
      } run;
#pragma unroll
      for (int j = 0; j < kEmitBases / 4; j++) {
        const uint32_t b = uint32_t(o >> (2 * (k - 4 * (j + 1)))) & 0xFFu;
        run.w[j] = (b >> 6) | (((b >> 4) & 3u) << 8) | (((b >> 2) & 3u) << 16) | ((b & 3u) << 24);
      }
      *reinterpret_cast<Run*>(at) = run;
    }
  }
  if (tail) {
    for (int i = writer ? kEmitBases : 0; i < k; i++) at[i] = uint8_t((o >> (2 * (k - 1 - i))) & 3);
  }
}

template <typename KeyT, int kEmitBases>
__global__ __launch_bounds__(256) void k_emit(DevSet<KeyT> set, const uint32_t* __restrict__ head,
                                               const uint32_t* __restrict__ pos,
                                               const uint8_t* __restrict__ ori,
                                               const UnitigPlace* __restrict__ place_at_head,
                                               uint8_t* __restrict__ bytes) {
  __shared__ int64_t s_bucket[2];
  const int64_t t = int64_t(blockIdx.x) * blockDim.x + threadIdx.x;
  set.block_bucket(s_bucket);
  if (t >= set.n) return;
  constexpr uint32_t kMask = uint32_t(kEmitBases - 1);
  const uint32_t p = pos[t], ob = ori[t];
  if ((p & kMask) != 0 && ((ob >> 1) & kMask) != 0) return;
  const uint32_t h = head[t];
  if (h == kNone) return;
  const UnitigPlace pl = place_at_head[h];
  const uint32_t flip = pl.flags & 1;
  const uint32_t q = flip ? (pl.len - 1 - p) : p;
  const bool tail = (pl.flags & 2) && q == pl.len - 1;
  const bool writer = (q & kMask) == 0;
  if (!writer && !tail) return;
  const uint64_t x = set.kmer_from_block(t, s_bucket);
  const uint64_t o = ((ob & 1u) ^ flip) ? revcomp(x, set.k) : x;
  store_bases<kEmitBases>(bytes + pl.base + q, o, set.k, writer, tail);
}

template <int kRun>
__device__ __forceinline__ void store_run(uint8_t* __restrict__ at, uint64_t o, int k, int first) {
  struct __attribute__((packed, aligned(1))) Run {
    uint32_t w[kRun / 4];
  } run;
#pragma unroll
  for (int j = 0; j < kRun / 4; j++) {
    const uint32_t b = uint32_t(o >> (2 * (k - first - 4 * (j + 1)))) & 0xFFu;
    run.w[j] = (b >> 6) | (((b >> 4) & 3u) << 8) | (((b >> 2) & 3u) << 16) | ((b & 3u) << 24);
  }
  *reinterpret_cast<Run*>(at + first) = run;
}
template <int kRun>
__device__ __forceinline__ void store_kmer(uint8_t* __restrict__ at, uint64_t o, int k) {
  if (kRun == 0) {
    for (int i = 0; i < k; i++) at[i] = uint8_t((o >> (2 * (k - 1 - i))) & 3);
  } else {
    store_run<(kRun ? kRun : 4)>(at, o, k, 0);
    if (k > kRun) store_run<(kRun ? kRun : 4)>(at, o, k, k - kRun);
  }
}

template <typename KeyT, int kRun>
__device__ __forceinline__ void emit_walk(const DevSet<KeyT>& set, const uint32_t* __restrict__ link,
                                          uint32_t first_state, uint2 own, uint64_t x_first,
                                          const UnitigPlace& pl, uint32_t q, uint8_t* __restrict__ bytes) {
  const int k = set.k;
  uint32_t cur = first_state;
  uint2 pr = own;
  uint64_t x = x_first;
  int since = 0;
  while (true) {
    const bool tail = (pl.flags & 2) && q == pl.len - 1;
    if (since == 0 || tail) {
      if (cur != first_state) x = set.kmer(cur >> 1);
      store_kmer<kRun>(bytes + pl.base + q, (cur & 1) ? revcomp(x, k) : x, k);
    }
    const uint32_t lk = leave_link(pr, cur);
    if (lk == kNone) return;
    cur = step_to(cur, lk);
    q++;
    since = since + 1 == k ? 0 : since + 1;
    if (sampled_ruler(cur) || q >= pl.len) return;
    pr = link_pair(link, cur);
  }
}

template <typename KeyT, int kRun>
__global__ __launch_bounds__(256) void k_emit_rulers(DevSet<KeyT> set, const uint32_t* __restrict__ link,
                                                      const unsigned long long* __restrict__ rinfo,
                                                      const unsigned long long* __restrict__ chain_info,
                                                      bool directed,
                                                      const UnitigPlace* __restrict__ place_at_head,
                                                      uint8_t* __restrict__ bytes) {
  __shared__ int64_t s_bucket[2];
  set.block_bucket_at((int64_t(blockIdx.x) * blockDim.x) << kRulerShift, s_bucket);
  const int64_t t = (int64_t(blockIdx.x) * blockDim.x + threadIdx.x) << kRulerShift;
  if (t >= set.n) return;
  const uint2 own = reinterpret_cast<const uint2*>(link)[t];
  Chosen c;
  if (!choose_at(uint32_t(t), own, rinfo, chain_info, directed, &c)) return;
  const UnitigPlace pl = place_at_head[c.head_state >> 1];
  const uint32_t flip = pl.flags & 1;
  emit_walk<KeyT, kRun>(set, link, 2 * uint32_t(t) + (c.d ^ flip), own, set.kmer_from_block(t, s_bucket), pl,
                        flip ? (c.len - 1 - c.p) : c.p, bytes);
}

template <typename KeyT, int kRun>
__global__ __launch_bounds__(256) void k_emit_heads(DevSet<KeyT> set, const uint32_t* __restrict__ link,
                                                     const unsigned long long* __restrict__ rinfo,
                                                     const unsigned long long* __restrict__ chain_info,
                                                     bool directed, const uint32_t* __restrict__ ends,
                                                     int64_t n_ends,
                                                     const UnitigPlace* __restrict__ place_at_head,
                                                     uint8_t* __restrict__ bytes) {
  const int64_t e = int64_t(blockIdx.x) * blockDim.x + threadIdx.x;
  if (e >= n_ends) return;
  const int64_t t = ends[e];
  if ((t & (kRulerEvery - 1)) == 0) return;
  const uint2 own = reinterpret_cast<const uint2*>(link)[t];
  Chosen c;
  if (!choose_at(uint32_t(t), own, rinfo, chain_info, directed, &c)) return;
  const UnitigPlace pl = place_at_head[c.head_state >> 1];
  const uint32_t flip = pl.flags & 1;
  const uint32_t first_state = 2 * uint32_t(t) + (c.d ^ flip);
  if (enter_link(own, first_state) != kNone) return;
  emit_walk<KeyT, kRun>(set, link, first_state, own, set.kmer(t), pl, flip ? (c.len - 1 - c.p) : c.p, bytes);
}

constexpr uint32_t kLongHead = 0x80000000u;
constexpr int kLongBlocks = 128;

template <typename KeyT, int kRun, bool kLongPass>
__device__ __forceinline__ void emit_logged(const DevSet<KeyT>& set, const uint32_t* __restrict__ link,
                                            const WalkLog& log, int64_t w, uint64_t hdr, uint32_t u,
                                            uint64_t x_u, const Chosen& c, const UnitigPlace& pl,
                                            uint8_t* __restrict__ bytes) {
  const int k = set.k;
  const uint32_t flip = pl.flags & 1;
  const uint32_t q_u = flip ? (c.len - 1 - c.p) : c.p;
  const bool with_string = (u & 1) == (c.d ^ flip);
  const uint32_t steps = uint32_t(hdr >> 32), arrival = uint32_t(hdr);
  const auto emit = [&](uint32_t state, uint32_t step, uint64_t x) {
    const uint32_t q = with_string ? q_u + step : q_u - step;
    if (q >= pl.len) return;
    const uint32_t as_read = with_string ? state : state ^ 1;
    store_kmer<kRun>(bytes + pl.base + q, (as_read & 1) ? revcomp(x, k) : x, k);
  };
  if (!kLongPass) {
    if (log.is_long(steps)) return;
    emit(u, 0, x_u);
    if (steps == 0) return;
    const int n_passed = int((steps - 1) / uint32_t(k));
    for (int j = 0; j < n_passed; j++) {
      const uint32_t st = log.mid[int64_t(j) * log.n_walkers + w];
      emit(st, uint32_t(j + 1) * uint32_t(k), set.kmer(st >> 1));
    }
    if (!sampled_ruler(arrival)) emit(arrival, steps, set.kmer(arrival >> 1));
  } else {
    emit(u, 0, x_u);
    uint32_t cur = u, step = 0;
    int since = 0;
    while (step < steps) {
      const uint32_t lk = leave_link(link_pair(link, cur), cur);
      if (lk == kNone) return;
      cur = step_to(cur, lk);
      step++;
      if (++since == k || step == steps) {
        since = 0;
        emit(cur, step, set.kmer(cur >> 1));
      }
    }
  }
}

template <typename KeyT, int kRun, bool kLongPass>
__device__ __forceinline__ void emit_ruler_walker(const DevSet<KeyT>& set, const uint32_t* __restrict__ link,
                                                  const unsigned long long* __restrict__ rinfo,
                                                  const WalkLog& log, bool directed, int64_t i, uint64_t x_t,
                                                  const UnitigPlace* __restrict__ place_at_head,
                                                  uint8_t* __restrict__ bytes) {
  const uint64_t hdr = log.hdr[i];
  bool self_only = false;
  if (hdr == kRecUnset) {
    if (kLongPass || (i & 1) || log.hdr[i ^ 1] != kRecUnset) return;
    self_only = true;
  }
  const int64_t t = (i >> 1) << kRulerShift;
  const ulonglong2 ri = reinterpret_cast<const ulonglong2*>(rinfo)[i >> 1];
  const Chosen c = choose_from_ends(uint32_t(ri.x), uint32_t((ri.x >> 32) & 0x7FFFFFFFu), uint32_t(ri.y),
                                    uint32_t((ri.y >> 32) & 0x7FFFFFFFu), directed);
  if (self_only) {
    const UnitigPlace pl = place_at_head[c.head_state >> 1];
    const uint32_t flip = pl.flags & 1;
    const uint32_t q = flip ? (c.len - 1 - c.p) : c.p;
    if (q < pl.len) store_kmer<kRun>(bytes + pl.base + q, ((c.d ^ flip) & 1) ? revcomp(x_t, set.k) : x_t, set.k);
    return;
  }
  emit_logged<KeyT, kRun, kLongPass>(set, link, log, i, hdr, uint32_t(2 * t + (i & 1)), x_t, c,
                                     place_at_head[c.head_state >> 1], bytes);
}

template <typename KeyT, int kRun, bool kLongPass>
__device__ __forceinline__ void emit_head_walker(const DevSet<KeyT>& set, const uint32_t* __restrict__ link,
                                                 const unsigned long long* __restrict__ rinfo,
                                                 const unsigned long long* __restrict__ chain_info,
                                                 const WalkLog& log, bool directed, const uint32_t* __restrict__ ends,
                                                 int64_t e, const UnitigPlace* __restrict__ place_at_head,
                                                 uint8_t* __restrict__ bytes) {
  const uint64_t hdr = log.hdr[e];
  if (hdr == kRecUnset) return;
  const uint32_t t = ends[e];
  const uint2 own = reinterpret_cast<const uint2*>(link)[t];
  Chosen c;
  if (!choose_at(t, own, rinfo, chain_info, directed, &c)) return;
  const uint32_t u = (own.y == kNone && own.x != kNone) ? 2 * t + 1 : 2 * t;
  emit_logged<KeyT, kRun, kLongPass>(set, link, log, e, hdr, u, set.kmer(t), c, place_at_head[c.head_state >> 1],
                                     bytes);
}

template <typename KeyT, int kRun>
__global__ __launch_bounds__(256) void k_emit_log_rulers(DevSet<KeyT> set, const uint32_t* __restrict__ link,
                                                          const unsigned long long* __restrict__ rinfo,
                                                          const unsigned long long* __restrict__ chain_info,
                                                          WalkLog log, WalkLog log_heads, bool directed,
                                                          const uint32_t* __restrict__ ends,
                                                          const UnitigPlace* __restrict__ place_at_head,
                                                          uint8_t* __restrict__ bytes) {
  __shared__ int64_t s_bucket[2];
  if (blockIdx.x < kLongBlocks) {
    const unsigned int n_long = *log.long_count;
    for (unsigned int at = blockIdx.x * blockDim.x + threadIdx.x; at < n_long; at += kLongBlocks * blockDim.x) {
      const uint32_t w = log.long_walkers[at];
      if (w & kLongHead) {
        emit_head_walker<KeyT, kRun, true>(set, link, rinfo, chain_info, log_heads, directed, ends,
                                           int64_t(w & ~kLongHead), place_at_head, bytes);
      } else {
        emit_ruler_walker<KeyT, kRun, true>(set, link, rinfo, log, directed, int64_t(w),
                                            set.kmer((int64_t(w) >> 1) << kRulerShift), place_at_head, bytes);
      }
    }
    return;
  }
  const int64_t first = int64_t(blockIdx.x - kLongBlocks) * blockDim.x;
  set.block_bucket_at((first >> 1) << kRulerShift, s_bucket);
  const int64_t i = first + threadIdx.x;
  if (i >= log.n_walkers || ((i >> 1) << kRulerShift) >= set.n) return;
  emit_ruler_walker<KeyT, kRun, false>(set, link, rinfo, log, directed, i,
                                       set.kmer_from_block((i >> 1) << kRulerShift, s_bucket), place_at_head, bytes);
}

template <typename KeyT, int kRun>
__global__ __launch_bounds__(256) void k_emit_log_heads(DevSet<KeyT> set, const uint32_t* __restrict__ link,
                                                         const unsigned long long* __restrict__ rinfo,
                                                         const unsigned long long* __restrict__ chain_info,
                                                         WalkLog log, bool directed,
                                                         const uint32_t* __restrict__ ends,
                                                         const UnitigPlace* __restrict__ place_at_head,
                                                         uint8_t* __restrict__ bytes) {
  const int64_t e = int64_t(blockIdx.x) * blockDim.x + threadIdx.x;
  if (e >= log.n_walkers) return;
  emit_head_walker<KeyT, kRun, false>(set, link, rinfo, chain_info, log, directed, ends, e, place_at_head, bytes);
}

__global__ __launch_bounds__(256) void k_pack(const uint8_t* __restrict__ bytes, int64_t n_bases,
                                               int64_t n_words, uint64_t* __restrict__ words) {
  const int64_t w = int64_t(blockIdx.x) * blockDim.x + threadIdx.x;
  if (w >= n_words) return;
  const int64_t p0 = w * 32;
  uint64_t out = 0;
  if (p0 + 32 <= n_bases) {
    const uint4 lo = *reinterpret_cast<const uint4*>(bytes + p0);
    const uint4 hi = *reinterpret_cast<const uint4*>(bytes + p0 + 16);
    const uint32_t q[8] = {lo.x, lo.y, lo.z, lo.w, hi.x, hi.y, hi.z, hi.w};
#pragma unroll
    for (int i = 0; i < 8; i++) {
#pragma unroll
      for (int b = 0; b < 4; b++) {
        const uint64_t code = (q[i] >> (8 * b)) & 3;
        out |= code << (62 - 2 * (4 * i + b));
      }
    }
  } else {
    for (int j = 0; j < 32 && p0 + j < n_bases; j++) out |= uint64_t(bytes[p0 + j] & 3) << (62 - 2 * j);
  }
  words[w] = out;
}

constexpr int kJumpRoundsMax = 48;
constexpr int kMatchBatch = 8;
constexpr int kMatchFirst = 4;
constexpr int kWalkRoundsMax = 40;
struct EncCtl {
  int64_t tot[3 + kLenSums];
  int self_rc;
  int rc_marks;
  int64_t t2[2];
  int64_t n_bases;
  unsigned long long sc_used;
  unsigned int long_count[2];
  int rc_batched;
  int tgt_extra;
  int jump_live[kJumpRoundsMax + 1];
  int match_live[kMatchBatch + 1];
  int walk_live[kWalkRoundsMax + 1];
};

struct EncPlan {
  int64_t n = 0, n_u = 0, n_strings = 0, n_bases = 0;
  int mode = 0;
  ksh_geom g{};
  ksh_set_view set{};
  uint32_t *nbr = nullptr, *link = nullptr, *head = nullptr, *pos = nullptr, *hlen = nullptr,
           *hlast = nullptr, *uid = nullptr;
  unsigned long long* info = nullptr;
  uint8_t *ori = nullptr, *hcls = nullptr;
  int64_t *c01 = nullptr, *c23 = nullptr;
  uint32_t* fine = nullptr;
  int fine_bits = 0;
  uint32_t* coarse = nullptr;
  char* ublock = nullptr;
  uint32_t *u_head = nullptr, *u_first = nullptr, *u_last = nullptr, *u_len = nullptr,
           *edges = nullptr, *mate = nullptr, *best_w = nullptr, *u_sid = nullptr,
           *u_koff = nullptr, *lens = nullptr, *sc_nodes = nullptr, *sc_parent = nullptr,
           *sc_rank = nullptr;
  unsigned long long *best_prio = nullptr, *sc_used = nullptr;
  uint8_t *visited = nullptr, *scls = nullptr, *u_flip = nullptr;
  int64_t *s_nk = nullptr, *sc01 = nullptr, *sc2 = nullptr, *str_start = nullptr;
  EncCtl* ctl = nullptr;
  int rounds = 0;
  int64_t routes = 0;
  bool stamped = true;
  bool directed = false;
  const unsigned long long *rinfo = nullptr, *chain_info = nullptr;
  const uint32_t* ends = nullptr;
  int64_t n_ends = 0;
  WalkLog log_rulers{}, log_heads{};
  bool cover = false;
  ksh_spss_view in{};
  int64_t* in_start = nullptr;
  bool ready = false;
  bool written = false;
  bool ambiguous = false;
};

inline size_t al(size_t x) { return (x + 255) & ~size_t(255); }

#define KSH_BOUND(cond)                                                                              \
  do {                                                                                               \
    if (!(cond)) return ::ksh::fail(KSH_INTERNAL, "encode: bound violated: %s (%s:%d)", #cond, __FILE__, __LINE__); \
  } while (0)
static_assert(sizeof(RcRecord<uint16_t>) == 8 && sizeof(RcRecord<uint32_t>) == 8 && sizeof(RcRecord<uint64_t>) == 16,
              "record sizes the scratch layout assumes");

constexpr int64_t kRcRowsMax = 512;
constexpr int64_t kRcWindowBytes = 78 << 10;

inline bool staged_adjacency() {
  static const bool on = [] {
    const char* e = getenv("KSH_ADJACENCY");
    return !(e && std::string(e) == "probe");
  }();
  return on;
}
inline bool rank_with_stamps() {
  static const bool on = [] {
    const char* e = getenv("KSH_RANK");
    return e && std::string(e) == "stamp";
  }();
  return on;
}
inline bool emit_by_walking() {
  static const bool on = [] {
    const char* e = getenv("KSH_EMIT");
    return e && std::string(e) == "walk";
  }();
  return on;
}
inline int64_t l2_threshold() {
  static const int64_t v = [] {
    const char* e = getenv("KSH_L2_MIN");
    return e ? std::max<int64_t>(4096, atoll(e)) : int64_t(1) << 20;
  }();
  return v;
}
inline unsigned nblk(int64_t n) { return unsigned(std::max<int64_t>(1, (n + 255) / 256)); }

template <typename T>
T* carve(char*& at, size_t count) {
  T* p = reinterpret_cast<T*>(at);
  at += al(count * sizeof(T));
  return p;
}

void free_plan(ksh_ctx* ctx) {
  EncPlan* p = static_cast<EncPlan*>(ctx->enc_state);
  if (!p) return;
  if (p->ublock) pool_free(ctx, p->ublock);
  delete p;
  ctx->enc_state = nullptr;
}

static bool replaces_unwritten(const ksh_ctx* ctx, bool cover) {
  const EncPlan* o = static_cast<const EncPlan*>(ctx->enc_state);
  return o && o->ready && !o->written && o->cover == cover;
}

void retire_plan(ksh_ctx* ctx) {
  if (EncPlan* p = static_cast<EncPlan*>(ctx->enc_state)) p->ready = false;
}

static int enc_fine_bits(const ksh_geom* g, int64_t n) {
  const int64_t nb = n_buckets(g);
  int fine_bits = 0;
  while (fine_bits < 13 && fine_bits + 2 < key_bits(g) && (int64_t(3) << fine_bits) < 2 * (n / nb + 1)) fine_bits++;
  return fine_bits;
}
static size_t enc_slot_bytes(const ksh_geom* g, int64_t n) {
  const int64_t nb = n_buckets(g);
  const int fine_bits = enc_fine_bits(g, n);
  const size_t fine_entries = fine_bits >= 2 ? (size_t(nb) << fine_bits) + 1 : 0;
  return 2 * al(size_t(2 * n) * 4) + al(size_t(2 * n) * 8) + 5 * al(size_t(n) * 4) + 2 * al(size_t(n)) +
         2 * al(size_t(n) * 8) + al(fine_entries * 4) + al(size_t((n >> kCoarseShift) + 2) * 4) +
         al(sizeof(EncCtl) + size_t(2 * nb) * 4) + 4096;
}
static size_t enc_arena_bytes(const ksh_geom* g, int64_t n) {
  const int64_t nb = n_buckets(g);
  return size_t(n / 256 + 4096) * 8 * 2 + (1u << 16) + size_t(n / kHeadSpan + 64) * 8 +
         (nb <= (1 << 14) ? size_t(kRcRowsMax) * 2 * nb * 4 + size_t(2 * nb + 1) * 16 + size_t(2 * nb) * 280 + 8192 : 0);
}
size_t encode_scratch_bytes(const ksh_geom* g, int64_t n) {
  const size_t slot = enc_slot_bytes(g, n), arena = enc_arena_bytes(g, n);
  return slot + (slot >> 3) + arena + (arena >> 2) + (size_t(2) << 20);
}
int encode_reserve(ksh_ctx* ctx, const ksh_geom* g, int64_t n) {
  KSH_TRY(slot_reserve(ctx, kSlotEncode, enc_slot_bytes(g, n)));
  return arena_reserve(ctx, enc_arena_bytes(g, n));
}

static int cover_stage(ksh_ctx* ctx, EncPlan* p, int64_t n_u, bool directed, bool slow, int k, int* walk_rounds_out) {
  hipStream_t st = ctx->stream;
  EncCtl* ctl = p->ctl;
  int walk_rounds = 0;
  p->rounds = 0;
  if (slow) {
    hipLaunchKernelGGL(k_match_slow, dim3(1), dim3(64), 0, st, p->edges, p->mate, n_u);
  } else {
    for (bool more = true; more;) {
      if (p->rounds) KSH_HIP(hipMemsetAsync(ctl->match_live, 0, sizeof(ctl->match_live), st));
      const int batch = p->rounds ? kMatchBatch : kMatchFirst;
      for (int r = 0; r < batch; r++) {
        hipLaunchKernelGGL(k_match_best, dim3(nblk(2 * n_u)), dim3(256), 0, st, p->edges, p->mate, 2 * n_u, directed,
                           p->best_prio, p->best_w, r ? &ctl->match_live[r - 1] : nullptr, &ctl->match_live[r]);
        hipLaunchKernelGGL(k_match_commit, dim3(nblk(2 * n_u)), dim3(256), 0, st, p->best_prio, p->best_w, 2 * n_u,
                           &ctl->match_live[r], p->mate);
      }
      KSH_HIP(hipMemcpyAsync(ctx->h_pinned, ctl->match_live, batch * sizeof(int), hipMemcpyDeviceToHost, st));
      KSH_HIP(hipStreamSynchronize(st));
      const int* live = reinterpret_cast<const int*>(ctx->h_pinned);
      int ran = 0;
      while (ran < batch && live[ran]) ran++;
      more = ran == batch;
      p->rounds += more ? batch : ran + 1;
      if (p->rounds > 100000) return fail(KSH_INTERNAL, "matching did not converge");
    }
    DevDsu dsu{reinterpret_cast<unsigned long long*>(p->sc01)};
    uint8_t* has_terminal = p->scls;
    hipLaunchKernelGGL(k_dsu_init, dim3(nblk(n_u)), dim3(256), 0, st, dsu.a, n_u, has_terminal);
    hipLaunchKernelGGL(k_dsu_unite_mates, dim3(nblk(2 * n_u)), dim3(256), 0, st, dsu, p->mate, 2 * n_u);
    hipLaunchKernelGGL(k_dsu_mark_terminals, dim3(nblk(n_u)), dim3(256), 0, st, dsu, p->mate, n_u, has_terminal);
    hipLaunchKernelGGL(k_dsu_open_paths, dim3(nblk(n_u)), dim3(256), 0, st, dsu, has_terminal, n_u, p->visited);
    hipLaunchKernelGGL(k_loop_cut, dim3(unsigned((n_u + 63) / 64)), dim3(64), 0, st, p->mate, n_u,
                       directed, p->visited, p->sc_nodes, p->sc_parent, p->sc_rank, p->sc_used);
  }
  unsigned long long* walk = p->best_prio;
  uint32_t* sid_at = p->best_w;
  hipLaunchKernelGGL(k_walk_init, dim3(nblk(2 * n_u)), dim3(256), 0, st, p->mate, p->u_len, 2 * n_u, walk);
  walk_rounds = 3;
  for (int64_t x = 2 * n_u; x > 1; x /= (kJumpHops + 1)) walk_rounds++;
  walk_rounds = std::min(walk_rounds, kWalkRoundsMax);
  for (int round = 0; round < walk_rounds; round++)
    hipLaunchKernelGGL(k_walk_jump, dim3(nblk(2 * n_u)), dim3(256), 0, st, 2 * n_u, walk,
                       round ? &ctl->walk_live[round - 1] : nullptr, &ctl->walk_live[round]);
  hipLaunchKernelGGL(k_string_starts, dim3(nblk(n_u)), dim3(256), 0, st, p->mate, p->u_len, walk, n_u,
                     directed, p->scls, p->s_nk, p->str_start);
  hipLaunchKernelGGL(k_string_counts, dim3(nblk(n_u)), dim3(256), 0, st, p->scls, n_u, slow, p->sc01,
                     p->sc2);
  arena_reset(ctx);
  int64_t* d_t2 = ctl->t2;
  KSH_TRY(scan_exclusive_i64(ctx, p->sc01, p->sc01, n_u, d_t2));
  KSH_TRY(scan_exclusive_i64(ctx, p->sc2, p->sc2, n_u, d_t2 + 1));
  hipLaunchKernelGGL(k_string_ids, dim3(nblk(n_u)), dim3(256), 0, st, n_u, p->scls, p->sc01, p->sc2, p->s_nk, d_t2,
                     slow, k, sid_at, p->lens, p->str_start);
  hipLaunchKernelGGL(k_string_assign, dim3(nblk(n_u)), dim3(256), 0, st, p->u_len, walk, n_u, p->scls, sid_at,
                     slow, p->u_sid, p->u_koff, p->u_flip, &ctl->walk_live[walk_rounds - 1]);
  *walk_rounds_out = walk_rounds;
  return KSH_OK;
}

template <typename KeyT>
int encode_plan_t(ksh_ctx* ctx, const ksh_geom* g, const ksh_set_view* sv, bool directed, int mode,
                  int64_t* n_strings, int64_t* n_bases) {
  const bool ambiguous = replaces_unwritten(ctx, false);
  free_plan(ctx);
  EncPlan* p = new EncPlan;
  ctx->enc_state = p;
  p->ambiguous = ambiguous;
  p->g = *g;
  p->set = *sv;
  p->mode = mode;
  const int64_t n = sv->n_keys;
  p->n = n;
  if (n == 0) {
    p->ready = true;
    *n_strings = 0;
    *n_bases = 0;
    return KSH_OK;
  }
  if (n >= int64_t(0x7FFFFFF0)) return fail(KSH_INVALID_ARGUMENT, "set too large for 32-bit indices");
  const int64_t nb = n_buckets(g);
  const int fine_bits = enc_fine_bits(g, n);
  const bool use_fine = fine_bits >= 2;
  const size_t fine_entries = use_fine ? (size_t(nb) << fine_bits) + 1 : 0;
  KSH_TRY(encode_reserve(ctx, g, n));
  arena_reset(ctx);
  char* at = ctx->slot[kSlotEncode];
  p->nbr = carve<uint32_t>(at, size_t(2 * n));
  p->link = carve<uint32_t>(at, size_t(2 * n));
  p->info = carve<unsigned long long>(at, size_t(2 * n));
  p->head = carve<uint32_t>(at, size_t(n));
  p->pos = carve<uint32_t>(at, size_t(n));
  p->hlen = carve<uint32_t>(at, size_t(n));
  p->hlast = carve<uint32_t>(at, size_t(n));
  p->uid = carve<uint32_t>(at, size_t(n));
  p->ori = carve<uint8_t>(at, size_t(n));
  p->hcls = carve<uint8_t>(at, size_t(n));
  p->c01 = carve<int64_t>(at, size_t(2 * n));
  p->c23 = p->c01 + n;
  p->fine = use_fine ? carve<uint32_t>(at, fine_entries) : nullptr;
  p->coarse = n >= 4 * nb ? carve<uint32_t>(at, size_t((n >> kCoarseShift) + 2)) : nullptr;
  p->ctl = reinterpret_cast<EncCtl*>(carve<char>(at, sizeof(EncCtl) + size_t(2 * nb) * 4));
  uint32_t* rc_cursor = reinterpret_cast<uint32_t*>(p->ctl + 1);
  EncCtl* ctl = p->ctl;

  DevSet<KeyT> set{sv->d_offsets, static_cast<const KeyT*>(sv->d_keys), nb, n, g->k, key_bits(g)};
  hipStream_t st = ctx->stream;
  if (use_fine) {
    hipLaunchKernelGGL((k_fine_index<KeyT>), dim3(unsigned(nb)), dim3(256), size_t(4) << fine_bits, st, sv->d_offsets,
                       static_cast<const KeyT*>(sv->d_keys), key_bits(g), fine_bits, p->fine, nb);
    set.fine = p->fine;
    set.fine_bits = fine_bits;
    p->fine_bits = fine_bits;
  }
  if (p->coarse) {
    const int64_t n_entries = (n >> kCoarseShift) + 1;
    hipLaunchKernelGGL((k_coarse_index<KeyT>), dim3(nblk(n_entries)), dim3(256), 0, st, set, n_entries, p->coarse);
    set.coarse = p->coarse;
  }
  KSH_HIP(hipMemsetAsync(ctl, 0, sizeof(EncCtl) + size_t(2 * nb) * 4, st));
  int* self_rc_flag = &ctl->self_rc;
  {
    Timer timer(ctx, 3, n);
    const int nbits = g->n_bucket_bits;
    if (directed) {
      hipLaunchKernelGGL((k_adjacency<KeyT, true>), dim3(nblk(n)), dim3(256), 0, st, set, p->nbr, self_rc_flag);
    } else if (staged_adjacency() && nbits <= 14 && 2 * g->k >= nbits + 4 &&
               key_bits(g) >= nbits + 2 + (nbits & 1) &&
               n / nb <= 4 * ((kRcWindowBytes - 4 * kRcSegs) / int64_t(sizeof(KeyT) + 6))) {
      const int64_t rows = std::max<int64_t>(1, std::min<int64_t>(kRcRowsMax, (n + 16383) / 16384));
      const int64_t per_row = ((n + rows - 1) / rows + 1023) / 1024 * 1024;
      KSH_BOUND(rows >= 1 && rows <= kRcRowsMax && rows * per_row >= n);
      KSH_BOUND(size_t(n) * sizeof(RcRecord<KeyT>) <= al(size_t(2 * n) * 8));
      static const bool one_level = [] {
        const char* e = getenv("KSH_RC_SCATTER");
        return e && std::string(e) == "direct";
      }();
      static const bool half_groups = [] {
        const char* e = getenv("KSH_RC_GROUPS");
        return e && std::string(e) == "half";
      }();
      const bool two_level = n >= (int64_t(1) << (half_groups ? 12 : 20)) && nbits > kSgBits && nbits <= 16 && !one_level;
      const int extra = (half_groups && two_level && nbits == 14 && key_bits(g) >= 2 * ((nbits + 1 + 2 + 1) / 2)) ? 1 : 0;
      const int gbits = nbits + extra;
      const int64_t ng = int64_t(1) << gbits;
      uint32_t* hist = static_cast<uint32_t*>(arena_alloc(ctx, size_t(rows) * ng * 4));
      int64_t* totals = static_cast<int64_t*>(arena_alloc(ctx, size_t(ng + 1) * 8));
      int64_t* goff = static_cast<int64_t*>(arena_alloc(ctx, size_t(ng + 1) * 8));
      if (!hist || !totals || !goff) return fail(KSH_INTERNAL, "scratch arena too small");
      RcRecord<KeyT>* rec = reinterpret_cast<RcRecord<KeyT>*>(p->info);
      uint32_t* rc0 = p->link;
      uint32_t* rc1 = p->link + n;
      const size_t hist_lds = size_t(ng) * 4;
      {
        const uint32_t bit = 1u << (sizeof(KeyT) == 2 ? 0 : sizeof(KeyT) == 4 ? 1 : 2);
        if (!(ctx->lds_opt_in & bit)) {
          const int bytes = int(kRcWindowBytes + 2048);
          KSH_HIP(hipFuncSetAttribute(reinterpret_cast<const void*>(k_adj_rc<KeyT, 1024>),
                                      hipFuncAttributeMaxDynamicSharedMemorySize, bytes));
          KSH_HIP(hipFuncSetAttribute(reinterpret_cast<const void*>(k_adj_rc<KeyT, 512>),
                                      hipFuncAttributeMaxDynamicSharedMemorySize, bytes));
          KSH_HIP(hipFuncSetAttribute(reinterpret_cast<const void*>(k_adj_rc<KeyT, 256>),
                                      hipFuncAttributeMaxDynamicSharedMemorySize, bytes));
          KSH_HIP(hipFuncSetAttribute(reinterpret_cast<const void*>(k_adj_rc<KeyT, 64>),
                                      hipFuncAttributeMaxDynamicSharedMemorySize, bytes));
          KSH_HIP(hipFuncSetAttribute(reinterpret_cast<const void*>(k_adj_rc1<KeyT, 1024>),
                                      hipFuncAttributeMaxDynamicSharedMemorySize, kRc1LdsBytes));
          KSH_HIP(hipFuncSetAttribute(reinterpret_cast<const void*>(k_adj_rc1<KeyT, 512>),
                                      hipFuncAttributeMaxDynamicSharedMemorySize, kRc1LdsBytes));
          KSH_HIP(hipFuncSetAttribute(reinterpret_cast<const void*>(k_adj_rc1<KeyT, 256>),
                                      hipFuncAttributeMaxDynamicSharedMemorySize, kRc1LdsBytes));
          KSH_HIP(hipFuncSetAttribute(reinterpret_cast<const void*>(k_adj_rc1<KeyT, 64>),
                                      hipFuncAttributeMaxDynamicSharedMemorySize, kRc1LdsBytes));
          KSH_HIP(hipFuncSetAttribute(reinterpret_cast<const void*>(k_rc_hist<KeyT>),
                                      hipFuncAttributeMaxDynamicSharedMemorySize, int(size_t(4) << 15)));
          ctx->lds_opt_in |= bit;
        }
      }
      KSH_BOUND(hist_lds <= (size_t(4) << 15) && ng <= 65536);
      hipLaunchKernelGGL((k_rc_hist<KeyT>), dim3(unsigned(rows)), dim3(1024), hist_lds, st,
                         static_cast<const KeyT*>(sv->d_keys), n, g->k, key_bits(g), gbits, per_row, hist);
      hipLaunchKernelGGL(k_rc_columns, dim3(unsigned((ng + 63) / 64)), dim3(64 * kColTeams), 0, st, hist, rows, int(ng),
                         totals);
      KSH_TRY(scan_exclusive_i64(ctx, totals, goff, ng, goff + ng));
      p->routes |= KSH_ROUTE_PROBE_STAGED | (two_level ? KSH_ROUTE_SCATTER_TWO_LEVEL : 0);
      if (two_level) {
        RcRecord<KeyT>* tmp_rec = sizeof(RcRecord<KeyT>) == 8 ? rec + n : reinterpret_cast<RcRecord<KeyT>*>(p->nbr);
        uint16_t* tmp_g = reinterpret_cast<uint16_t*>(p->head);
        KSH_BOUND(sizeof(RcRecord<KeyT>) == 8 ? size_t(2 * n) * sizeof(RcRecord<KeyT>) <= al(size_t(2 * n) * 8)
                                    : reinterpret_cast<char*>(p->link) == reinterpret_cast<char*>(p->nbr) + al(size_t(2 * n) * 4) &&
                                          size_t(n) * sizeof(RcRecord<KeyT>) <= 2 * al(size_t(2 * n) * 4));
        KSH_BOUND(gbits - kSgBits <= 8);
        uint32_t* cursor = rc_cursor;
        constexpr int kPer = sizeof(RcRecord<KeyT>) == 8 ? 4 : 2;
        hipLaunchKernelGGL((k_rc_scatter_l1<KeyT, kPer>), dim3(unsigned(rows)), dim3(kL1Threads), 0, st, set, gbits,
                           per_row, hist, goff, tmp_rec, tmp_g);
        hipLaunchKernelGGL((k_rc_scatter_l2<KeyT>), dim3(unsigned((n + kL2Tile - 1) / kL2Tile)), dim3(kL2Threads), 0,
                           st, n, gbits, goff, tmp_rec, tmp_g, cursor, rec);
      } else {
        hipLaunchKernelGGL((k_rc_scatter<KeyT>), dim3(unsigned(rows)), dim3(1024), hist_lds, st, set, gbits, 0, 0,
                           per_row, hist, goff, rec);
      }
      const int64_t per_group = n / ng;
      const int cap = int(std::min<int64_t>((kRcWindowBytes - 4 * kRcSegs) / int64_t(sizeof(KeyT) + 6),
                                            std::max<int64_t>(1024, extra ? per_group * 23 / 20 + 256 : per_group * 5 / 4 + 256))) & ~7;
      const size_t rc_lds = size_t(cap) * (sizeof(KeyT) + 4) + size_t(cap + 2 * kRcSegs) * 2;
      KSH_BOUND(cap >= 8 && cap % 8 == 0 && cap + 2 * kRcSegs < 65536);
      KSH_BOUND(rc_lds + 2048 <= size_t(kRcWindowBytes) + 2048 && rc_lds <= size_t(kRcWindowBytes));
      int64_t* pb = static_cast<int64_t*>(arena_alloc(ctx, size_t(ng) * 2 * kRcSegs * 8));
      int64_t* pb0 = extra ? static_cast<int64_t*>(arena_alloc(ctx, size_t(ng) * 2 * 8)) : nullptr;
      if (!pb || (extra && !pb0)) return fail(KSH_INTERNAL, "scratch arena too small");
      hipLaunchKernelGGL((k_rc_bounds<KeyT>), dim3(nblk(ng * 2 * kRcSegs + (extra ? ng * 2 : 0))), dim3(256), 0, st, set,
                         gbits, pb, pb0);
      p->routes |= per_group > 4096 ? KSH_ROUTE_RC_1024 : per_group > 1024 ? KSH_ROUTE_RC_512
                   : per_group > 256 ? KSH_ROUTE_RC_256 : KSH_ROUTE_RC_64;
      static const int rc1_mode = [] {
        const char* e = getenv("KSH_RC1");
        return !e ? 1 : (std::string(e) == "marks" ? 2 : (std::string(e) == "batched" ? 0 : 1));
      }();
      const bool rc1_marks = rc1_mode == 2;
      const int rc1_cap = rc1_marks ? 0 : int(std::min<int64_t>(Rc1Cfg<KeyT>::kCap, (per_group * 4 / 3 + 263) & ~int64_t(7)));
      const int pass1_cap = rc1_marks ? -1 : rc1_cap;
      const bool with_rc = rc1_mode != 0;
      int rc1_sbits = 6;
      while ((1 << rc1_sbits) < kRc1SlicesMax && (2 << rc1_sbits) <= rc1_cap + 1) rc1_sbits++;
      const size_t rc1_lds = (size_t(4) << rc1_sbits) + size_t(rc1_cap) * Rc1Cfg<KeyT>::kEntryBytes;
      KSH_BOUND(rc1_lds <= size_t(kRc1LdsBytes) && rc1_cap % 8 == 0 && rc1_cap < (2 << rc1_sbits) - 1);
      if (!rc1_marks) p->routes |= KSH_ROUTE_RC1_STREAMED;
      const int rc1_batched = rc1_mode == 0 ? 1 : 0;
#define KSH_LAUNCH_RC(T)                                                                                              \
  do {                                                                                                                \
    if (with_rc)                                                                                                      \
      hipLaunchKernelGGL((k_adj_rc<KeyT, T>), dim3(unsigned(ng)), dim3(T), rc_lds, st, set, gbits, goff, rec, pb, pb0, \
                         cap, rc0, rc1, &ctl->rc_batched, pass1_cap, &ctl->rc_marks);                                 \
    if (!rc1_marks)                                                                                                   \
      hipLaunchKernelGGL((k_adj_rc1<KeyT, T>), dim3(unsigned(ng)), dim3(T), rc1_lds, st, set, gbits, goff, rec, pb,   \
                         pb0, rc1_cap, rc1_sbits, rc1_batched, rc0, rc1, &ctl->rc_batched);                           \
  } while (0)
      if (per_group > 4096)
        KSH_LAUNCH_RC(1024);
      else if (per_group > 1024)
        KSH_LAUNCH_RC(512);
      else if (per_group > 256)
        KSH_LAUNCH_RC(256);
      else
        KSH_LAUNCH_RC(64);
#undef KSH_LAUNCH_RC
      static const int fwd_mode = [] {
        const char* e = getenv("KSH_FWD");
        return !e ? 0 : (std::string(e) == "probe" ? 1 : (std::string(e) == "staged" ? 2 : 0));
      }();
      if (fwd_mode == 1) {
        hipLaunchKernelGGL((k_adj_fwd<KeyT>), dim3(nblk(n)), dim3(256), 0, st, set, rc0, rc1, p->nbr, self_rc_flag);
      } else if (fwd_mode == 0) {
        p->routes |= KSH_ROUTE_FWD_TARGETS;
        constexpr int kTgtChunk = TgtCfg<KeyT>::kChunk, kTgtStreamMax = TgtCfg<KeyT>::kStreamMax;
        const int64_t n_chunks = (n + kTgtChunk - 1) / kTgtChunk;
        const int64_t cap = n / kTgtStreamMax + 1;
        const size_t cut_bytes = size_t((n_chunks + 1) * kTgtBounds + (n_chunks + cap) * 2 * kTgtBounds) * 8 + size_t(cap) * sizeof(TgtTask);
        int64_t* cuts = cut_bytes <= al(size_t(2 * n) * 8) ? reinterpret_cast<int64_t*>(p->info)
                                                           : static_cast<int64_t*>(arena_alloc(ctx, cut_bytes));
        if (!cuts) return fail(KSH_INTERNAL, "scratch arena too small");
        int64_t* rec = cuts + (n_chunks + 1) * kTgtBounds;
        TgtTask* task = reinterpret_cast<TgtTask*>(rec + (n_chunks + cap) * 2 * kTgtBounds);
        KSH_BOUND(n_chunks >= 1 && n_chunks * kTgtChunk >= n && n < (int64_t(1) << 31));
        hipLaunchKernelGGL((k_tgt_bounds<KeyT>), dim3(nblk((n_chunks + 1) * 8)), dim3(256), 0, st, set, n_chunks, cuts);
        hipLaunchKernelGGL(k_tgt_split, dim3(nblk(n_chunks)), dim3(256), 0, st, cuts, n_chunks, cap, kTgtStreamMax, rec, task,
                           &ctl->tgt_extra);
        hipLaunchKernelGGL((k_tgt_subcuts<KeyT>), dim3(nblk(cap * 8)), dim3(256), 0, st, set, cuts, n_chunks, cap, task,
                           &ctl->tgt_extra, rec);
        hipLaunchKernelGGL((k_adj_fwd_targets<KeyT>), dim3(unsigned(n_chunks + cap)), dim3(kTgtThreads), 0, st, set, rec,
                           n_chunks, &ctl->tgt_extra, rc0, rc1, p->nbr, self_rc_flag);
      } else {
        p->routes |= KSH_ROUTE_FWD_STAGED;
        const int64_t n_chunks = (n + kFwdChunk - 1) / kFwdChunk;
        int64_t* bounds = reinterpret_cast<int64_t*>(p->info);
        KSH_BOUND(size_t(n_chunks + 1) * kFwdBounds * 8 <= al(size_t(2 * n) * 8));
        hipLaunchKernelGGL((k_fwd_bounds<KeyT>), dim3(nblk((n_chunks + 1) * 10)), dim3(256), 0, st, set, n_chunks, bounds);
        hipLaunchKernelGGL((k_adj_fwd_staged<KeyT>), dim3(unsigned(n_chunks)), dim3(kFwdChunk), 0, st, set, bounds,
                           rc0, rc1, p->nbr, self_rc_flag);
#ifdef KSH_FWD_DEBUG
        {
          unsigned long long h[8];
          (void)hipStreamSynchronize(st);
          (void)hipMemcpyFromSymbol(h, HIP_SYMBOL(g_fwd_dbg), sizeof(h));
          fprintf(stderr, "fwd dbg: kmers %llu next!usable %llu next-bucket-miss %llu prev!usable %llu prev-bucket-miss %llu "
                          "next-range>cap %llu two-top-bases %llu\n", h[0], h[1], h[2], h[3], h[4], h[5], h[6]);
          unsigned long long z[8] = {};
          (void)hipMemcpyToSymbol(HIP_SYMBOL(g_fwd_dbg), z, sizeof(z));
        }
#endif
      }
    } else {
      hipLaunchKernelGGL((k_adjacency<KeyT, false>), dim3(nblk(n)), dim3(256), 0, st, set, p->nbr, self_rc_flag);
    }
  }
  if (directed)
    hipLaunchKernelGGL((k_link_cut<KeyT, true>), dim3(nblk(n)), dim3(256), 0, st, set, p->nbr);
  else
    hipLaunchKernelGGL((k_link_cut<KeyT, false>), dim3(nblk(n)), dim3(256), 0, st, set, p->nbr);
  const uint32_t* link = p->nbr;
  const int64_t n_hblocks = (n + kHeadSpan - 1) / kHeadSpan;
  int64_t* b01 = p->c23;
  int64_t* b23 = p->c23 + n_hblocks;
  int64_t* d_tot = ctl->tot;
  int64_t* end_before = static_cast<int64_t*>(arena_alloc(ctx, size_t(n_hblocks + 1) * 8));
  if (!end_before) return fail(KSH_INTERNAL, "scratch arena too small");
  uint32_t* ends = p->pos;
  uint8_t* end_flags = p->ori;
  KSH_BOUND(size_t(n_hblocks) * 256 <= al(size_t(n)));
  hipLaunchKernelGGL(k_end_counts, dim3(unsigned(n_hblocks)), dim3(256), 0, st, link, n, end_before, end_flags);
  KSH_TRY(scan_exclusive_i64(ctx, end_before, end_before, n_hblocks, end_before + n_hblocks));
  hipLaunchKernelGGL(k_end_fill, dim3(unsigned(n_hblocks)), dim3(256), 0, st, end_flags, n, end_before, ends, p->hcls);
  p->directed = directed;
  p->ends = ends;
  KSH_HIP(hipMemcpyAsync(ctx->h_pinned, end_before + n_hblocks, 8, hipMemcpyDeviceToHost, st));
  KSH_HIP(hipStreamSynchronize(st));
  const int64_t n_ends = ctx->h_pinned[0];
  p->n_ends = n_ends;
  for (bool stamped = rank_with_stamps(), first_pass = true;; stamped = true, first_pass = false) {
    const int64_t ns2 = 2 * n;
    const int64_t n_dense = 2 * ((n + kRulerEvery - 1) / kRulerEvery);
    unsigned long long* rinfo = stamped ? reinterpret_cast<unsigned long long*>(p->c01) : p->info;
    unsigned long long* chain_info = stamped ? reinterpret_cast<unsigned long long*>(p->c23) : p->info + n_dense;
    {
      Timer timer(ctx, 4, n);
      if (stamped) {
        KSH_HIP(hipMemsetAsync(p->info, 0xFF, size_t(2 * n) * 8, st));
        hipLaunchKernelGGL(k_ruler_walk, dim3(nblk(n_dense)), dim3(256), 0, st, link, ns2, n_dense, rinfo, p->info);
        hipLaunchKernelGGL(k_ruler_heads, dim3(nblk(n_ends)), dim3(256), 0, st, link, ends, n_ends, p->info, chain_info);
      } else {
        WalkLog lr{}, lh{};
        lr.k = lh.k = g->k;
        const size_t used = (size_t(n_dense) + size_t(n)) * 8;
        const size_t log_bytes = size_t(n_dense) * (8 + 4 * kLogMidRulers + 4) + size_t(n_ends) * (8 + 4 * kLogMidHeads + 4) + 64;
        if (!emit_by_walking() && used + log_bytes <= size_t(2 * n) * 8) {
          unsigned long long* at8 = p->info + n_dense + n;
          lr.hdr = at8;
          lh.hdr = at8 + n_dense;
          uint32_t* at4 = reinterpret_cast<uint32_t*>(at8 + n_dense + n_ends);
          lr.mid = at4;
          lh.mid = at4 + size_t(kLogMidRulers) * n_dense;
          lr.long_walkers = lh.long_walkers = lh.mid + size_t(kLogMidHeads) * n_ends;
          lr.long_count = lh.long_count = ctl->long_count;
          lr.long_tag = 0;
          lh.long_tag = kLongHead;
          lr.n_walkers = n_dense;
          lh.n_walkers = n_ends;
          lr.n_mid = kLogMidRulers;
          lh.n_mid = kLogMidHeads;
          KSH_HIP(hipMemsetAsync(at8, 0xFF, size_t(n_dense + n_ends) * 8, st));
          p->routes |= KSH_ROUTE_EMIT_LOGS;
        }
        p->log_rulers = lr;
        p->log_heads = lh;
        KSH_HIP(hipMemsetAsync(rinfo, 0xFF, size_t(n_dense) * 8, st));
        hipLaunchKernelGGL(k_rank_unset, dim3(nblk(n_ends)), dim3(256), 0, st, ends, n_ends, chain_info);
        static const int64_t race_min = [] {
          const char* e = getenv("KSH_RANK_PHASES");
          if (e && std::string(e) == "1") return int64_t(0);
          if (e && std::string(e) == "2") return int64_t(1) << 60;
          const char* m = getenv("KSH_RANK_RACE_MIN");
          return m ? int64_t(atoll(m)) : int64_t(1) << 18;
        }();
        p->routes |= (n_dense >= race_min ? KSH_ROUTE_RANK_ONE_LAUNCH : 0) | (n_ends >= race_min ? KSH_ROUTE_HEADS_ONE_LAUNCH : 0);
        if (n_dense < race_min)
          hipLaunchKernelGGL(k_rank_walk<1>, dim3(nblk(n_dense)), dim3(256), 0, st, link, ns2, n_dense, rinfo, chain_info, lr,
                             static_cast<unsigned long long*>(nullptr), static_cast<unsigned long long*>(nullptr));
        if (n_ends < race_min)
          hipLaunchKernelGGL(k_rank_heads<1>, dim3(nblk(n_ends)), dim3(256), 0, st, link, ends, n_ends, rinfo, chain_info, lh);
        const bool l2_after = n_dense >= l2_threshold();
        hipLaunchKernelGGL(k_rank_walk<2>, dim3(nblk(n_dense)), dim3(256), 0, st, link, ns2, n_dense, rinfo, chain_info, lr,
                           l2_after ? reinterpret_cast<unsigned long long*>(p->hlen) : nullptr,
                           l2_after ? reinterpret_cast<unsigned long long*>(p->hlast) : nullptr);
        hipLaunchKernelGGL(k_rank_heads<2>, dim3(nblk(n_ends)), dim3(256), 0, st, link, ends, n_ends, rinfo, chain_info, lh);
      }
    }
    const bool two_levels = !stamped && n_dense >= l2_threshold();
    const int64_t n_jump = two_levels ? (((n_dense - 1) >> (kL2Shift + 1)) << 1) + 2 : n_dense;
    unsigned long long* r2 = reinterpret_cast<unsigned long long*>(p->uid);
    unsigned long long* l2_head = reinterpret_cast<unsigned long long*>(p->hlen);
    unsigned long long* l2_stamp = reinterpret_cast<unsigned long long*>(p->hlast);
    if (two_levels) p->routes |= KSH_ROUTE_JUMP_TWO_LEVEL;
    if (stamped) p->routes = (p->routes | KSH_ROUTE_RANK_STAMPED) & ~int64_t(KSH_ROUTE_EMIT_LOGS | KSH_ROUTE_RANK_ONE_LAUNCH | KSH_ROUTE_HEADS_ONE_LAUNCH | KSH_ROUTE_JUMP_TWO_LEVEL);
    if (two_levels) {
      hipLaunchKernelGGL(k_l2_walk<true>, dim3(nblk(n_jump)), dim3(256), 0, st, rinfo, n_dense, r2, l2_head, l2_stamp);
      hipLaunchKernelGGL(k_l2_walk<false>, dim3(nblk(n_dense)), dim3(256), 0, st, rinfo, n_dense, r2, l2_head, l2_stamp);
    }
    int max_rounds = 3;
    for (int64_t x = n_jump; x > 1; x /= (kJumpHops + 1)) max_rounds++;
    max_rounds = std::min(max_rounds, kJumpRoundsMax);
    if (!first_pass) {
      KSH_HIP(hipMemsetAsync(ctl->jump_live, 0, sizeof(ctl->jump_live), st));
      KSH_HIP(hipMemsetAsync(d_tot, 0, (3 + kLenSums) * 8, st));
      KSH_HIP(hipMemsetAsync(ctl->long_count, 0, sizeof(ctl->long_count), st));
    }
    for (int round = 0; round < max_rounds; round++) {
      const int* prev = round ? &ctl->jump_live[round - 1] : nullptr;
      if (two_levels)
        hipLaunchKernelGGL(k_l2_jump, dim3(nblk(n_jump)), dim3(256), 0, st, n_jump, r2, prev, &ctl->jump_live[round]);
      else
        hipLaunchKernelGGL(k_ruler_jump, dim3(nblk(n_dense)), dim3(256), 0, st, n_dense, rinfo, prev,
                           &ctl->jump_live[round]);
    }
    if (two_levels)
      hipLaunchKernelGGL(k_l2_resolve, dim3(nblk(n_dense)), dim3(256), 0, st, n_dense, r2, l2_head, l2_stamp, rinfo);
    int* loop_flag = reinterpret_cast<int*>(d_tot + 2 + kLenSums);
    if (stamped) {
      hipLaunchKernelGGL(k_choose, dim3(nblk(n)), dim3(256), 0, st, p->info, rinfo, chain_info, n, directed,
                         p->head, p->pos, p->ori, p->hcls, p->hlen, p->hlast);
      hipLaunchKernelGGL(k_loops, dim3(nblk(n)), dim3(256), 0, st, link, n, p->head, p->pos, p->ori,
                         p->hcls, p->hlen, p->hlast);
    } else {
      hipLaunchKernelGGL(k_choose_ends, dim3(nblk(n_ends)), dim3(256), 0, st, link, ends, n_ends, rinfo, chain_info,
                         directed, p->head, p->ori, p->hcls, p->hlen, p->hlast,
                         reinterpret_cast<unsigned long long*>(d_tot + 2), loop_flag);
      hipLaunchKernelGGL(k_rulers_done, dim3(nblk(n_dense)), dim3(256), 0, st, rinfo, n_dense, loop_flag);
    }
    hipLaunchKernelGGL(k_head_block_counts, dim3(unsigned(n_hblocks)), dim3(256), 0, st, p->hcls, n, b01, b23);
    KSH_TRY(scan_exclusive_i64(ctx, b01, b01, n_hblocks, d_tot));
    KSH_TRY(scan_exclusive_i64(ctx, b23, b23, n_hblocks, d_tot + 1));
    KSH_HIP(hipGetLastError());
    static_assert(offsetof(EncCtl, self_rc) == (3 + kLenSums) * 8 && (4 + kLenSums) <= 64, "one copy: tot + self_rc");
    KSH_HIP(hipMemcpyAsync(ctx->h_pinned, d_tot, (4 + kLenSums) * 8, hipMemcpyDeviceToHost, st));
    KSH_HIP(hipStreamSynchronize(st));
    if (*reinterpret_cast<int*>(ctx->h_pinned + 3 + kLenSums))
      return fail(KSH_INVALID_ARGUMENT, "the canonical set holds a k-mer that is its own reverse "
                                        "complement (even k): not supported");
    static_assert(offsetof(EncCtl, rc_marks) == offsetof(EncCtl, self_rc) + 4, "the word behind self_rc, in the same copy");
    if (reinterpret_cast<int*>(ctx->h_pinned + 3 + kLenSums)[1]) p->routes |= KSH_ROUTE_RC_MARKS_GROUPS;
    p->stamped = stamped;
    p->rinfo = rinfo;
    p->chain_info = chain_info;
    if (stamped) break;
    int64_t accounted = 0;
    for (int i = 0; i < kLenSums; i++) accounted += ctx->h_pinned[2 + i];
    if (accounted == n && *reinterpret_cast<int*>(ctx->h_pinned + 2 + kLenSums) == 0) break;
  }
  const int64_t n0 = ctx->h_pinned[0] & 0xFFFFFFFF, n1 = ctx->h_pinned[0] >> 32;
  const int64_t n2 = ctx->h_pinned[1] & 0xFFFFFFFF, n3 = ctx->h_pinned[1] >> 32;
  const int64_t n_u = n0 + n1 + n2 + n3;
  p->n_u = n_u;

  const size_t ub = 10 * al(size_t(n_u) * 4) + al(size_t(8 * n_u) * 4) + 2 * al(size_t(2 * n_u) * 4) +
                    al(size_t(2 * n_u) * 8) + 3 * al(size_t(n_u)) + 4 * al(size_t(n_u + 1) * 8) +
                    3 * al(size_t(n_u) * 4) + 4096;
  KSH_TRY(pool_alloc(ctx, ub, reinterpret_cast<void**>(&p->ublock)));
  at = p->ublock;
  p->u_head = carve<uint32_t>(at, size_t(n_u));
  p->u_first = carve<uint32_t>(at, size_t(n_u));
  p->u_last = carve<uint32_t>(at, size_t(n_u));
  p->u_len = carve<uint32_t>(at, size_t(n_u));
  p->u_sid = carve<uint32_t>(at, size_t(n_u));
  p->u_koff = carve<uint32_t>(at, size_t(n_u));
  p->lens = carve<uint32_t>(at, size_t(n_u));
  p->sc_nodes = carve<uint32_t>(at, size_t(n_u));
  p->sc_parent = carve<uint32_t>(at, size_t(n_u));
  p->sc_rank = carve<uint32_t>(at, size_t(n_u));
  p->edges = carve<uint32_t>(at, size_t(8 * n_u));
  p->mate = carve<uint32_t>(at, size_t(2 * n_u));
  p->best_w = carve<uint32_t>(at, size_t(2 * n_u));
  p->best_prio = carve<unsigned long long>(at, size_t(2 * n_u));
  p->visited = carve<uint8_t>(at, size_t(n_u));
  p->scls = carve<uint8_t>(at, size_t(n_u));
  p->u_flip = carve<uint8_t>(at, size_t(n_u));
  p->s_nk = carve<int64_t>(at, size_t(n_u + 1));
  p->sc01 = carve<int64_t>(at, size_t(n_u + 1));
  p->sc2 = carve<int64_t>(at, size_t(n_u + 1));
  p->str_start = carve<int64_t>(at, size_t(n_u + 1));
  p->sc_used = &ctl->sc_used;

  hipLaunchKernelGGL(k_unitig_fill, dim3(unsigned(n_hblocks)), dim3(256), 0, st, p->hcls, b01, b23, n, n0,
                     n0 + n1, n0 + n1 + n2, p->ori, p->hlen, p->hlast, p->uid, p->u_head, p->u_first,
                     p->u_last, p->u_len);

  int64_t ns = n_u;
  int walk_rounds = 0;
  if (mode == 1) {
    hipLaunchKernelGGL(k_unitig_strings, dim3(nblk(n_u)), dim3(256), 0, st, p->u_len, n_u, g->k,
                       p->u_sid, p->u_koff, p->u_flip, p->lens, p->str_start);
  } else {
    hipLaunchKernelGGL((k_edges<KeyT>), dim3(nblk(2 * n_u)), dim3(256), 0, st, set, 2 * n_u, directed,
                       p->u_first, p->u_last, p->head, p->uid, p->edges, p->mate);
    KSH_TRY(cover_stage(ctx, p, n_u, directed, mode == 2, g->k, &walk_rounds));
  }
  arena_reset(ctx);
  KSH_TRY(scan_exclusive_i64(ctx, p->str_start, p->str_start, n_u, &ctl->n_bases));
  hipLaunchKernelGGL(k_unitig_place, dim3(nblk(n_u)), dim3(256), 0, st, p->u_len, p->u_sid, p->u_koff,
                     p->u_flip, p->str_start, p->lens, p->u_head, n_u, reinterpret_cast<UnitigPlace*>(p->c01),
                     walk_rounds > 0 ? &ctl->walk_live[walk_rounds - 1] : nullptr);
  KSH_HIP(hipGetLastError());
  constexpr size_t kTail = sizeof(EncCtl) - offsetof(EncCtl, t2);
  static_assert(kTail <= 64 * sizeof(int64_t) && offsetof(EncCtl, n_bases) == offsetof(EncCtl, t2) + 16, "pinned read-back");
  KSH_HIP(hipMemcpyAsync(ctx->h_pinned, ctl->t2, kTail, hipMemcpyDeviceToHost, st));
  KSH_HIP(hipStreamSynchronize(st));
  const int* walk_live_host = reinterpret_cast<const int*>(reinterpret_cast<const char*>(ctx->h_pinned) +
                                                           (offsetof(EncCtl, walk_live) - offsetof(EncCtl, t2)));
  if (walk_rounds > 0 && walk_live_host[walk_rounds - 1])
    return fail(KSH_INTERNAL, "the path cover still holds a loop");
  {
    const char* tail = reinterpret_cast<const char*>(ctx->h_pinned);
    const auto at_tail = [&](size_t member_off) { return tail + (member_off - offsetof(EncCtl, t2)); };
    if (*reinterpret_cast<const int*>(at_tail(offsetof(EncCtl, rc_batched)))) p->routes |= KSH_ROUTE_RC_BATCHED;
    if (*reinterpret_cast<const int*>(at_tail(offsetof(EncCtl, tgt_extra))) > 0) p->routes |= KSH_ROUTE_TGT_PARTS;
    const unsigned int* lc = reinterpret_cast<const unsigned int*>(at_tail(offsetof(EncCtl, long_count)));
    if (!p->stamped && (lc[0] || lc[1])) p->routes |= KSH_ROUTE_LONG_STRETCHES;
    if (p->rounds > kMatchFirst) p->routes |= KSH_ROUTE_MATCH_MORE_ROUNDS;
  }
  if (mode != 1) ns = (ctx->h_pinned[0] & 0xFFFFFFFF) + (ctx->h_pinned[0] >> 32) + ctx->h_pinned[1];
  p->n_strings = ns;
  p->n_bases = ctx->h_pinned[2];
  p->ready = true;
  *n_strings = p->n_strings;
  *n_bases = p->n_bases;
  return KSH_OK;
}

template <typename KeyT>
int encode_write_t(ksh_ctx* ctx, uint64_t* d_words, uint32_t* d_lens) {
  EncPlan* p = static_cast<EncPlan*>(ctx->enc_state);
  if (p->n == 0) return KSH_OK;
  const ksh_geom* g = &p->g;
  const int64_t n = p->n;
  DevSet<KeyT> set{p->set.d_offsets, static_cast<const KeyT*>(p->set.d_keys), n_buckets(g), n, g->k,
                   key_bits(g)};
  set.fine = p->fine;
  set.fine_bits = p->fine_bits;
  set.coarse = p->coarse;
  hipStream_t st = ctx->stream;
  const size_t need = size_t(p->n_bases) + 64;
  uint8_t* bytes;
  void* tmp = nullptr;
  if (need <= size_t(2 * n) * 4) {
    bytes = reinterpret_cast<uint8_t*>(p->link);
  } else {
    KSH_TRY(pool_alloc(ctx, need, &tmp));
    bytes = static_cast<uint8_t*>(tmp);
  }
  {
    Timer timer(ctx, 5, n);
    const UnitigPlace* place = reinterpret_cast<const UnitigPlace*>(p->c01);
    const int64_t n_sampled = (n + kRulerEvery - 1) / kRulerEvery;
#define KSH_EMIT(W, R)                                                                                         \
  do {                                                                                                         \
    if (p->stamped) {                                                                                          \
      hipLaunchKernelGGL((k_emit<KeyT, W>), dim3(nblk(n)), dim3(256), 0, st, set, p->head, p->pos, p->ori,     \
                         place, bytes);                                                                        \
    } else if (p->log_rulers.hdr) {                                                                            \
      hipLaunchKernelGGL((k_emit_log_rulers<KeyT, R>), dim3(kLongBlocks + nblk(p->log_rulers.n_walkers)),      \
                         dim3(256), 0, st, set, p->nbr, p->rinfo, p->chain_info, p->log_rulers, p->log_heads,  \
                         p->directed, p->ends, place, bytes);                                                  \
      hipLaunchKernelGGL((k_emit_log_heads<KeyT, R>), dim3(nblk(p->log_heads.n_walkers)), dim3(256), 0, st,    \
                         set, p->nbr, p->rinfo, p->chain_info, p->log_heads, p->directed, p->ends, place,      \
                         bytes);                                                                               \
    } else {                                                                                                   \
      hipLaunchKernelGGL((k_emit_rulers<KeyT, R>), dim3(nblk(n_sampled)), dim3(256), 0, st, set, p->nbr,       \
                         p->rinfo, p->chain_info, p->directed, place, bytes);                                  \
      hipLaunchKernelGGL((k_emit_heads<KeyT, R>), dim3(nblk(p->n_ends)), dim3(256), 0, st, set, p->nbr,        \
                         p->rinfo, p->chain_info, p->directed, p->ends, p->n_ends, place, bytes);              \
    }                                                                                                          \
  } while (0)
    if (g->k >= 16)
      KSH_EMIT(16, 16);
    else if (g->k >= 8)
      KSH_EMIT(4, 8);
    else if (g->k >= 4)
      KSH_EMIT(4, 4);
    else
      KSH_EMIT(1, 0);
#undef KSH_EMIT
  }
  const int64_t n_words = (p->n_bases + 31) / 32;
  hipLaunchKernelGGL(k_pack, dim3(nblk(n_words)), dim3(256), 0, st, bytes, p->n_bases, n_words,
                     d_words);
  KSH_HIP(hipMemcpyAsync(d_lens, p->lens, size_t(p->n_strings) * 4, hipMemcpyDeviceToDevice, st));
  KSH_HIP(hipGetLastError());
  if (tmp) pool_free(ctx, tmp);
  return KSH_OK;
}

constexpr int64_t kCoverMaxStrings = (int64_t(1) << 30) - 1;
int cover_plan(ksh_ctx* ctx, const ksh_geom* g, const ksh_spss_view* in, bool directed, bool slow,
               int64_t* n_strings, int64_t* n_bases) {
  const bool ambiguous = replaces_unwritten(ctx, true);
  free_plan(ctx);
  EncPlan* p = new EncPlan;
  ctx->enc_state = p;
  p->ambiguous = ambiguous;
  p->cover = true;
  p->g = *g;
  p->in = *in;
  p->directed = directed;
  p->mode = slow ? 2 : 0;
  const int64_t n = in->n_strings;
  p->n = n;
  p->n_u = n;
  if (n == 0) {
    p->ready = true;
    *n_strings = 0;
    *n_bases = 0;
    return KSH_OK;
  }
  const int k = g->k;
  const int n_tables = directed ? 2 : 1;
  uint64_t cap = 1;
  while (cap < uint64_t(4 * n)) cap <<= 1;
  const size_t block = al(sizeof(EncCtl)) + al(kCoverErrCount * 8 + 8) + 7 * al(size_t(n) * 4) +
                       al(size_t(8 * n) * 4) + 2 * al(size_t(2 * n) * 4) + al(size_t(2 * n) * 8) + 3 * al(size_t(n)) +
                       5 * al(size_t(n + 1) * 8) + 2 * al(size_t(n) * 8) + al(n_tables * cap * 8) +
                       al(n_tables * cap * 4) + 4096;
  KSH_TRY(arena_reserve(ctx, size_t(n / 256 + 4096) * 8 * 2 + (1u << 16)));
  KSH_TRY(pool_alloc(ctx, block, reinterpret_cast<void**>(&p->ublock)));
  char* at = p->ublock;
  p->ctl = reinterpret_cast<EncCtl*>(carve<char>(at, sizeof(EncCtl)));
  unsigned long long* err = carve<unsigned long long>(at, kCoverErrCount + 1);
  int64_t* in_total = reinterpret_cast<int64_t*>(err + kCoverErrCount);
  p->u_len = carve<uint32_t>(at, size_t(n));
  p->u_sid = carve<uint32_t>(at, size_t(n));
  p->u_koff = carve<uint32_t>(at, size_t(n));
  p->lens = carve<uint32_t>(at, size_t(n));
  p->sc_nodes = carve<uint32_t>(at, size_t(n));
  p->sc_parent = carve<uint32_t>(at, size_t(n));
  p->sc_rank = carve<uint32_t>(at, size_t(n));
  p->edges = carve<uint32_t>(at, size_t(8 * n));
  p->mate = carve<uint32_t>(at, size_t(2 * n));
  p->best_w = carve<uint32_t>(at, size_t(2 * n));
  p->best_prio = carve<unsigned long long>(at, size_t(2 * n));
  p->visited = carve<uint8_t>(at, size_t(n));
  p->scls = carve<uint8_t>(at, size_t(n));
  p->u_flip = carve<uint8_t>(at, size_t(n));
  p->s_nk = carve<int64_t>(at, size_t(n + 1));
  p->sc01 = carve<int64_t>(at, size_t(n + 1));
  p->sc2 = carve<int64_t>(at, size_t(n + 1));
  p->str_start = carve<int64_t>(at, size_t(n + 1));
  p->in_start = carve<int64_t>(at, size_t(n + 1));
  uint64_t* first = carve<uint64_t>(at, size_t(n));
  uint64_t* last = carve<uint64_t>(at, size_t(n));
  unsigned long long* keys = carve<unsigned long long>(at, n_tables * cap);
  uint32_t* vals = carve<uint32_t>(at, n_tables * cap);
  KSH_BOUND(size_t(at - p->ublock) <= block);
  p->sc_used = &p->ctl->sc_used;
  EncCtl* ctl = p->ctl;
  hipStream_t st = ctx->stream;

  KSH_HIP(hipMemsetAsync(ctl, 0, sizeof(EncCtl), st));
  KSH_HIP(hipMemsetAsync(err, 0xFF, kCoverErrCount * 8, st));
  KSH_HIP(hipMemsetAsync(keys, 0xFF, n_tables * cap * 8, st));
  arena_reset(ctx);
  cover_launch_sizes(st, in->d_lens, n, k, p->in_start);
  KSH_TRY(scan_exclusive_i64(ctx, p->in_start, p->in_start, n, in_total));
  cover_launch_ends(st, in, p->in_start, in_total, k, directed, first, last, keys, vals, cap, err);
  KSH_HIP(hipGetLastError());
  KSH_HIP(hipMemcpyAsync(ctx->h_pinned, err, (kCoverErrCount + 1) * 8, hipMemcpyDeviceToHost, st));
  KSH_HIP(hipStreamSynchronize(st));
  const unsigned long long* e = reinterpret_cast<const unsigned long long*>(ctx->h_pinned);
  if (e[kCoverErrBases] != ~0ull)
    return fail(KSH_INVALID_ARGUMENT, "cover: the strings' lengths (lens + K) add up to %lld bases, not n_bases = %lld",
                (long long)ctx->h_pinned[kCoverErrCount], (long long)in->n_bases);
  if (e[kCoverErrPalindrome] != ~0ull)
    return fail(KSH_INVALID_ARGUMENT, "cover: an end k-mer of string %llu is its own reverse complement (even k): "
                                      "not supported", e[kCoverErrPalindrome]);
  if (e[kCoverErrSameEnds] != ~0ull)
    return fail(KSH_INVALID_ARGUMENT, "cover: string %llu is longer than K and its first and last k-mers have the "
                                      "same canonical form", e[kCoverErrSameEnds]);
  if (e[kCoverErrDupEnd] != ~0ull)
    return fail(KSH_INVALID_ARGUMENT, "cover: an end k-mer of string %llu is, up to reverse complement, an end "
                                      "k-mer of another string too (a string given twice, or with its reverse "
                                      "complement)", e[kCoverErrDupEnd]);
  if (e[kCoverErrDupFirst] != ~0ull)
    return fail(KSH_INVALID_ARGUMENT, "cover: the first k-mer of string %llu is the first k-mer of another string "
                                      "too (repeated first k-mer)", e[kCoverErrDupFirst]);
  if (e[kCoverErrDupLast] != ~0ull)
    return fail(KSH_INVALID_ARGUMENT, "cover: the last k-mer of string %llu is the last k-mer of another string "
                                      "too (repeated last k-mer)", e[kCoverErrDupLast]);

  cover_launch_edges(st, first, last, in->d_lens, n, k, directed, keys, vals, cap, p->u_len, p->edges, p->mate);
  int walk_rounds = 0;
  KSH_TRY(cover_stage(ctx, p, n, directed, slow, k, &walk_rounds));
  arena_reset(ctx);
  KSH_TRY(scan_exclusive_i64(ctx, p->str_start, p->str_start, n, &ctl->n_bases));
  KSH_HIP(hipGetLastError());
  constexpr size_t kTail = sizeof(EncCtl) - offsetof(EncCtl, t2);
  KSH_HIP(hipMemcpyAsync(ctx->h_pinned, ctl->t2, kTail, hipMemcpyDeviceToHost, st));
  KSH_HIP(hipStreamSynchronize(st));
  const int* walk_live_host = reinterpret_cast<const int*>(reinterpret_cast<const char*>(ctx->h_pinned) +
                                                           (offsetof(EncCtl, walk_live) - offsetof(EncCtl, t2)));
  if (walk_live_host[walk_rounds - 1]) return fail(KSH_INTERNAL, "the path cover still holds a loop");
  p->n_strings = (ctx->h_pinned[0] & 0xFFFFFFFF) + (ctx->h_pinned[0] >> 32) + ctx->h_pinned[1];
  p->n_bases = ctx->h_pinned[2];
  p->ready = true;
  *n_strings = p->n_strings;
  *n_bases = p->n_bases;
  return KSH_OK;
}

int cover_write(ksh_ctx* ctx, uint64_t* d_words, uint32_t* d_lens) {
  EncPlan* p = static_cast<EncPlan*>(ctx->enc_state);
  if (p->n == 0) return KSH_OK;
  hipStream_t st = ctx->stream;
  void* tmp = nullptr;
  KSH_TRY(pool_alloc(ctx, size_t(p->n_bases) + 64, &tmp));
  uint8_t* bytes = static_cast<uint8_t*>(tmp);
  cover_launch_emit(st, &p->in, p->in_start, p->u_len, p->u_sid, p->u_koff, p->u_flip, p->str_start, p->g.k,
                    p->n_bases, bytes);
  const int64_t n_words = (p->n_bases + 31) / 32;
  hipLaunchKernelGGL(k_pack, dim3(nblk(n_words)), dim3(256), 0, st, bytes, p->n_bases, n_words, d_words);
  KSH_HIP(hipMemcpyAsync(d_lens, p->lens, size_t(p->n_strings) * 4, hipMemcpyDeviceToDevice, st));
  KSH_HIP(hipGetLastError());
  pool_free(ctx, tmp);
  return KSH_OK;
}
// ... 148 lines not shown
```

Before: 28200.

## Split interleaved neighbour array into two per-side link arrays

```diff
diff --git a/kmer-sets-compression_amd/csrc/ksh_encode.hip b/kmer-sets-compression_amd/csrc/ksh_encode.hip
--- a/kmer-sets-compression_amd/csrc/ksh_encode.hip
+++ b/kmer-sets-compression_amd/csrc/ksh_encode.hip
@@ -127,8 +127,8 @@
 }
 
 template <typename KeyT, bool kDirected>
-__global__ __launch_bounds__(256) void k_adjacency(DevSet<KeyT> set, uint32_t* __restrict__ nbr,
-                                                    int* __restrict__ self_rc) {
+__global__ __launch_bounds__(256) void k_adjacency(DevSet<KeyT> set, uint32_t* __restrict__ nbr0,
+                                                    uint32_t* __restrict__ nbr1, int* __restrict__ self_rc) {
   __shared__ int64_t s_bucket[2];
   const int64_t t = int64_t(blockIdx.x) * blockDim.x + threadIdx.x;
   const uint64_t x = set.kmer_in_block(t, s_bucket);
@@ -143,25 +143,25 @@
       cnt[side]++;
       single[side] = (uint32_t(idx) << 1) | same;
     });
-  nbr[2 * t] = cnt[0] == 0 ? kNone : (cnt[0] == 1 ? single[0] : kMulti);
-  nbr[2 * t + 1] = cnt[1] == 0 ? kNone : (cnt[1] == 1 ? single[1] : kMulti);
+  nbr0[t] = cnt[0] == 0 ? kNone : (cnt[0] == 1 ? single[0] : kMulti);
+  nbr1[t] = cnt[1] == 0 ? kNone : (cnt[1] == 1 ? single[1] : kMulti);
 }
 
 template <typename KeyT, bool kDirected>
-__global__ __launch_bounds__(256) void k_link_cut(DevSet<KeyT> set, uint32_t* __restrict__ nbr) {
+__global__ __launch_bounds__(256) void k_link_cut(DevSet<KeyT> set, uint32_t* nbr0, uint32_t* nbr1) {
   const int64_t t = int64_t(blockIdx.x) * blockDim.x + threadIdx.x;
   if (t >= set.n) return;
-  const uint2 mine = reinterpret_cast<const uint2*>(nbr)[t];
+  const uint2 mine = make_uint2(nbr0[t], nbr1[t]);
   if (mine.x != kMulti && mine.y != kMulti) return;
   const uint64_t x = set.kmer(t);
   const uint64_t rx = kDirected ? 0 : revcomp(x, set.k);
   for (int side = 0; side < 2; side++) {
     if ((side ? mine.y : mine.x) != kMulti) continue;
     for_side_neighbours<KeyT, kDirected>(set, x, rx, t, side, [&](int64_t idx, uint32_t same) {
-      uint32_t* facing = nbr + 2 * idx + (same ? side : side ^ 1);
+      uint32_t* facing = ((same ? side : side ^ 1) ? nbr1 : nbr0) + idx;
       if (*reinterpret_cast<volatile uint32_t*>(facing) < kMulti) *reinterpret_cast<volatile uint32_t*>(facing) = kNone;
     });
-    nbr[2 * t + side] = kNone;
+    (side ? nbr1 : nbr0)[t] = kNone;
   }
 }
 
@@ -951,9 +951,8 @@
 
 template <typename KeyT, int kFwdCapNext = FwdCfg<KeyT>::kCapNext>
 __global__ __launch_bounds__(kFwdChunk, (sizeof(KeyT) <= 4 ? 8 : 4)) void k_adj_fwd_staged(DevSet<KeyT> set, const int64_t* __restrict__ bounds,
-                                                              const uint32_t* __restrict__ rc0,
-                                                              const uint32_t* __restrict__ rc1,
-                                                              uint32_t* __restrict__ nbr,
+                                                              uint32_t* __restrict__ rc0,
+                                                              uint32_t* __restrict__ rc1,
                                                               int* __restrict__ self_rc) {
   constexpr int kFwdCapPrev = FwdCfg<KeyT>::kCapPrev;
   static_assert(kFwdCapNext % kFwdChunk == 0, "staging shape");
@@ -1139,7 +1138,8 @@
     const int total = cnt[side] + (r[side] == kNone ? 0 : (r[side] == kMulti ? 2 : 1));
     out[side] = total == 0 ? kNone : (total > 1 ? kMulti : (cnt[side] == 1 ? single[side] : r[side]));
   }
-  reinterpret_cast<uint2*>(nbr)[t] = make_uint2(out[0], out[1]);
+  rc0[t] = out[0];
+  rc1[t] = out[1];
   KSH_PMARK(0, 6);
 }
 
@@ -1278,9 +1278,8 @@
 template <typename KeyT>
 __global__ __launch_bounds__(kTgtThreads, 8) void k_adj_fwd_targets(DevSet<KeyT> set, const int64_t* __restrict__ rec,
                                                                    int64_t n_chunks, const int* __restrict__ n_extra,
-                                                                   const uint32_t* __restrict__ rc0,
-                                                                   const uint32_t* __restrict__ rc1,
-                                                                   uint32_t* __restrict__ nbr, int* __restrict__ self_rc) {
+                                                                   uint32_t* __restrict__ rc0,
+                                                                   uint32_t* __restrict__ rc1, int* __restrict__ self_rc) {
   constexpr int kRounds = (TgtCfg<KeyT>::kChunk + 3 + kTgtThreads - 1) / kTgtThreads;
   __shared__ KeyT s_keys[kRounds * kTgtThreads];
   __shared__ uint32_t s_slot[kRounds * kTgtThreads];
@@ -1400,7 +1399,7 @@
       });
     }
     const uint32_t direct = cnt == 0 ? kNone : (cnt == 1 ? single : kMulti);
-    nbr[2 * size_t(p32) + 1] = side_verdict(direct, through_rc);
+    rc1[p32] = side_verdict(direct, through_rc);
   }
   KSH_PMARK(0, 4);
   __syncthreads();
@@ -1408,7 +1407,7 @@
 #pragma unroll
   for (int u = 0; u < kRounds; u++) {
     const int i = tid + u * kTgtThreads;
-    if (i < len_w) nbr[2 * (b + i)] = s_slot[i];
+    if (i < len_w) rc0[b + i] = s_slot[i];
   }
   KSH_PMARK(0, 6);
 #ifdef KSH_TRACE
@@ -1417,9 +1416,8 @@
 }
 
 template <typename KeyT>
-__global__ __launch_bounds__(256) void k_adj_fwd(DevSet<KeyT> set, const uint32_t* __restrict__ rc0,
-                                                  const uint32_t* __restrict__ rc1,
-                                                  uint32_t* __restrict__ nbr, int* __restrict__ self_rc) {
+__global__ __launch_bounds__(256) void k_adj_fwd(DevSet<KeyT> set, uint32_t* __restrict__ rc0,
+                                                  uint32_t* __restrict__ rc1, int* __restrict__ self_rc) {
   __shared__ int64_t s_bucket[2];
   const int64_t t = int64_t(blockIdx.x) * blockDim.x + threadIdx.x;
   const uint64_t x = set.kmer_in_block(t, s_bucket);
@@ -1450,11 +1448,20 @@
     const int total = cnt[side] + (r[side] == kNone ? 0 : (r[side] == kMulti ? 2 : 1));
     out[side] = total == 0 ? kNone : (total > 1 ? kMulti : (cnt[side] == 1 ? single[side] : r[side]));
   }
-  reinterpret_cast<uint2*>(nbr)[t] = make_uint2(out[0], out[1]);
-}
-
-__device__ __forceinline__ uint2 link_pair(const uint32_t* __restrict__ link, uint32_t s) {
-  return reinterpret_cast<const uint2*>(link)[s >> 1];
+  rc0[t] = out[0];
+  rc1[t] = out[1];
+}
+
+struct Links {
+  const uint32_t* side0;
+  const uint32_t* side1;
+};
+__device__ __forceinline__ uint2 links_of(const Links& link, int64_t t) {
+  return make_uint2(link.side0[t], link.side1[t]);
+}
+__device__ __forceinline__ uint2 link_pair(const Links& link, uint32_t s) { return links_of(link, s >> 1); }
+__device__ __forceinline__ uint32_t leave_at(const Links& link, uint32_t s) {
+  return ((s & 1) ? link.side0 : link.side1)[s >> 1];
 }
 __device__ __forceinline__ uint32_t leave_link(uint2 pr, uint32_t s) { return (s & 1) ? pr.x : pr.y; }
 __device__ __forceinline__ uint32_t enter_link(uint2 pr, uint32_t s) { return (s & 1) ? pr.y : pr.x; }
@@ -1475,7 +1482,7 @@
   return (end ? kEndFlag : 0) | (uint64_t(dist & 0x7FFFFFFFu) << 32) | nx;
 }
 
-__global__ __launch_bounds__(256) void k_ruler_walk(const uint32_t* __restrict__ link,
+__global__ __launch_bounds__(256) void k_ruler_walk(Links link,
                                                      int64_t n_states, int64_t n_dense,
                                                      unsigned long long* __restrict__ rinfo,
                                                      unsigned long long* __restrict__ rec) {
@@ -1487,7 +1494,7 @@
     return;
   }
   const uint32_t r = uint32_t(s64);
-  uint32_t lk = leave_link(link_pair(link, r), r);
+  uint32_t lk = leave_at(link, r);
   if ((r & 1) == 0) rec[r] = make_rec(0, 0, uint32_t(i));
   if (lk == kNone) {
     rinfo[i] = make_rinfo(true, 0, r);
@@ -1502,7 +1509,7 @@
       return;
     }
     if ((cur & 1) == 0) rec[cur] = make_rec(0, steps, uint32_t(i));
-    lk = leave_link(link_pair(link, cur), cur);
+    lk = leave_at(link, cur);
     if (lk == kNone) {
       rinfo[i] = make_rinfo(true, steps, cur);
       return;
@@ -1514,7 +1521,7 @@
   return (ruler_ahead ? kEndFlag : 0) | (uint64_t(steps & 0x7FFFFFFFu) << 32) | ref;
 }
 
-__global__ __launch_bounds__(256) void k_ruler_heads(const uint32_t* __restrict__ link,
+__global__ __launch_bounds__(256) void k_ruler_heads(Links link,
                                                       const uint32_t* __restrict__ ends, int64_t n_ends,
                                                       unsigned long long* __restrict__ rec,
                                                       unsigned long long* __restrict__ chain_info) {
@@ -1522,13 +1529,13 @@
   if (e >= n_ends) return;
   const int64_t t = ends[e];
   if ((t & (kRulerEvery - 1)) == 0) return;
-  const uint2 own = reinterpret_cast<const uint2*>(link)[t];
+  const uint2 own = links_of(link, t);
   const uint32_t flags = (own.x == kNone ? 1u : 0u) | (own.y == kNone ? 2u : 0u);
   if (!flags) return;
   for (uint32_t d = 0; d < 2; d++) {
     if (!(flags & (1u << d))) continue;
     const uint32_t s0 = uint32_t(2 * t) | d;
-    uint32_t lk = leave_link(link_pair(link, s0), s0);
+    uint32_t lk = leave_at(link, s0);
     if (lk == kNone) {
       rec[s0] = make_rec(2, 0, s0);
       continue;
@@ -1542,7 +1549,7 @@
         chain_info[t] = make_chain_info(true, off, dense_index(cur));
         break;
       }
-      lk = leave_link(link_pair(link, cur), cur);
+      lk = leave_at(link, cur);
       if (lk == kNone || off >= 0x3FFFFFFFu) {
         if ((cur & 1) == 0) rec[cur] = make_rec(3, off, s0);
         chain_info[t] = make_chain_info(false, off, cur);
@@ -1584,7 +1591,7 @@
 constexpr int kLogMidRulers = 7, kLogMidHeads = 7;
 
 template <int kPhase>
-__global__ __launch_bounds__(256) void k_rank_walk(const uint32_t* __restrict__ link, int64_t n_states,
+__global__ __launch_bounds__(256) void k_rank_walk(Links link, int64_t n_states,
                                                     int64_t n_dense, unsigned long long* __restrict__ rinfo,
                                                     unsigned long long* __restrict__ chain_info, WalkLog log,
                                                     unsigned long long* __restrict__ unset_a,
@@ -1625,7 +1632,7 @@
       since = 0;
       log.passed(i, n_passed++, cur);
     }
-    lk = leave_link(link_pair(link, cur), cur);
+    lk = leave_at(link, cur);
     if (lk == kNone) {
       rec_post(rinfo + i, make_rinfo(true, steps, cur));
       rec_post(chain_info + (cur >> 1), make_chain_info(true, steps, dense_index(r ^ 1)));
@@ -1636,7 +1643,7 @@
 }
 
 template <int kPhase>
-__global__ __launch_bounds__(256) void k_rank_heads(const uint32_t* __restrict__ link,
+__global__ __launch_bounds__(256) void k_rank_heads(Links link,
                                                      const uint32_t* __restrict__ ends, int64_t n_ends,
                                                      unsigned long long* __restrict__ rinfo,
                                                      unsigned long long* __restrict__ chain_info, WalkLog log) {
@@ -1644,7 +1651,7 @@
   if (e >= n_ends) return;
   const uint32_t t = ends[e];
   if ((t & (kRulerEvery - 1)) == 0) return;
-  const uint2 own = reinterpret_cast<const uint2*>(link)[t];
+  const uint2 own = links_of(link, t);
   uint32_t s0;
   if (own.x == kNone && own.y != kNone) {
     s0 = 2 * t;
@@ -1672,7 +1679,7 @@
       since = 0;
       log.passed(e, n_passed++, cur);
     }
-    lk = leave_link(link_pair(link, cur), cur);
+    lk = leave_at(link, cur);
     if (lk == kNone || off >= 0x3FFFFFFFu) {
       rec_post(chain_info + t, make_chain_info(false, off, cur));
       rec_post(chain_info + (cur >> 1), make_chain_info(false, off, s0 ^ 1));
@@ -1924,7 +1931,7 @@
   return true;
 }
 
-__global__ __launch_bounds__(256) void k_choose_ends(const uint32_t* __restrict__ link,
+__global__ __launch_bounds__(256) void k_choose_ends(Links link,
                                                       const uint32_t* __restrict__ ends, int64_t n_ends,
                                                       const unsigned long long* __restrict__ rinfo,
                                                       const unsigned long long* __restrict__ chain_info,
@@ -1939,7 +1946,7 @@
   const int64_t e = int64_t(blockIdx.x) * blockDim.x + threadIdx.x;
   if (e < n_ends) {
     const uint32_t t = ends[e];
-    const uint2 own = reinterpret_cast<const uint2*>(link)[t];
+    const uint2 own = links_of(link, t);
     Chosen c;
     if (!choose_at(t, own, rinfo, chain_info, directed, &c)) {
       *loop_flag = 1;
@@ -1964,7 +1971,7 @@
   if (i < n_dense && !(rinfo[i] & kEndFlag)) *loop_flag = 1;
 }
 
-__global__ __launch_bounds__(256) void k_loops(const uint32_t* __restrict__ link,
+__global__ __launch_bounds__(256) void k_loops(Links link,
                                                 int64_t n, uint32_t* __restrict__ head,
                                                 uint32_t* __restrict__ pos,
                                                 uint8_t* __restrict__ ori,
@@ -1978,7 +1985,7 @@
   uint32_t s = start;
   int64_t steps = 0;
   do {
-    const uint32_t lk = link[s ^ 1];
+    const uint32_t lk = leave_at(link, s);
     if (lk == kNone) return;
     s = ((lk >> 1) << 1) | ((s & 1) ^ (lk & 1));
     if ((s >> 1) < uint32_t(t)) return;
@@ -1994,7 +2001,7 @@
     pos[y] = p;
     ori[y] = ori_byte(s & 1, len - 1 - p);
     last = s;
-    const uint32_t lk = link[s ^ 1];
+    const uint32_t lk = leave_at(link, s);
     s = ((lk >> 1) << 1) | ((s & 1) ^ (lk & 1));
     p++;
   } while (s != start);
@@ -2041,23 +2048,28 @@
   return before + inc;
 }
 
-__device__ __forceinline__ uint32_t end_flags8(const uint32_t* __restrict__ link, int64_t t0, int64_t n) {
+__device__ __forceinline__ uint32_t end_flags8(Links link, int64_t t0, int64_t n) {
   uint32_t flags = 0;
-#pragma unroll
-  for (int i = 0; i < kHeadItems; i += 2) {
-    if (t0 + i + 1 < n) {
-      const uint4 v = *reinterpret_cast<const uint4*>(link + 2 * (t0 + i));
+  if (t0 + kHeadItems <= n) {
+#pragma unroll
+    for (int i = 0; i < kHeadItems; i += 4) {
+      const uint4 a = *reinterpret_cast<const uint4*>(link.side0 + t0 + i);
+      const uint4 b = *reinterpret_cast<const uint4*>(link.side1 + t0 + i);
+      if (a.x == kNone || b.x == kNone) flags |= 1u << i;
+      if (a.y == kNone || b.y == kNone) flags |= 1u << (i + 1);
+      if (a.z == kNone || b.z == kNone) flags |= 1u << (i + 2);
+      if (a.w == kNone || b.w == kNone) flags |= 1u << (i + 3);
+    }
+  } else {
+    for (int i = 0; i < kHeadItems && t0 + i < n; i++) {
+      const uint2 v = links_of(link, t0 + i);
       if (v.x == kNone || v.y == kNone) flags |= 1u << i;
-      if (v.z == kNone || v.w == kNone) flags |= 1u << (i + 1);
-    } else if (t0 + i < n) {
-      const uint2 v = *reinterpret_cast<const uint2*>(link + 2 * (t0 + i));
-      if (v.x == kNone || v.y == kNone) flags |= 1u << i;
     }
   }
   return flags;
 }
 
-__global__ __launch_bounds__(256) void k_end_counts(const uint32_t* __restrict__ link, int64_t n,
+__global__ __launch_bounds__(256) void k_end_counts(Links link, int64_t n,
                                                      int64_t* __restrict__ counts, uint8_t* __restrict__ flags8) {
   __shared__ uint64_t lds4[4];
   const int64_t t0 = (int64_t(blockIdx.x) * 256 + threadIdx.x) * kHeadItems;
@@ -2646,12 +2658,12 @@
 }
 
 template <typename KeyT, int kRun>
-__device__ __forceinline__ void emit_walk(const DevSet<KeyT>& set, const uint32_t* __restrict__ link,
+__device__ __forceinline__ void emit_walk(const DevSet<KeyT>& set, Links link,
                                           uint32_t first_state, uint2 own, uint64_t x_first,
                                           const UnitigPlace& pl, uint32_t q, uint8_t* __restrict__ bytes) {
   const int k = set.k;
   uint32_t cur = first_state;
-  uint2 pr = own;
+  uint32_t lk = leave_link(own, cur);
   uint64_t x = x_first;
   int since = 0;
   while (true) {
@@ -2660,18 +2672,17 @@
       if (cur != first_state) x = set.kmer(cur >> 1);
       store_kmer<kRun>(bytes + pl.base + q, (cur & 1) ? revcomp(x, k) : x, k);
     }
-    const uint32_t lk = leave_link(pr, cur);
     if (lk == kNone) return;
     cur = step_to(cur, lk);
     q++;
     since = since + 1 == k ? 0 : since + 1;
     if (sampled_ruler(cur) || q >= pl.len) return;
-    pr = link_pair(link, cur);
+    lk = leave_at(link, cur);
   }
 }
 
 template <typename KeyT, int kRun>
-__global__ __launch_bounds__(256) void k_emit_rulers(DevSet<KeyT> set, const uint32_t* __restrict__ link,
+__global__ __launch_bounds__(256) void k_emit_rulers(DevSet<KeyT> set, Links link,
                                                       const unsigned long long* __restrict__ rinfo,
                                                       const unsigned long long* __restrict__ chain_info,
                                                       bool directed,
@@ -2681,7 +2692,7 @@
   set.block_bucket_at((int64_t(blockIdx.x) * blockDim.x) << kRulerShift, s_bucket);
   const int64_t t = (int64_t(blockIdx.x) * blockDim.x + threadIdx.x) << kRulerShift;
   if (t >= set.n) return;
-  const uint2 own = reinterpret_cast<const uint2*>(link)[t];
+  const uint2 own = links_of(link, t);
   Chosen c;
   if (!choose_at(uint32_t(t), own, rinfo, chain_info, directed, &c)) return;
   const UnitigPlace pl = place_at_head[c.head_state >> 1];
@@ -2691,7 +2702,7 @@
 }
 
 template <typename KeyT, int kRun>
-__global__ __launch_bounds__(256) void k_emit_heads(DevSet<KeyT> set, const uint32_t* __restrict__ link,
+__global__ __launch_bounds__(256) void k_emit_heads(DevSet<KeyT> set, Links link,
                                                      const unsigned long long* __restrict__ rinfo,
                                                      const unsigned long long* __restrict__ chain_info,
                                                      bool directed, const uint32_t* __restrict__ ends,
@@ -2702,7 +2713,7 @@
   if (e >= n_ends) return;
   const int64_t t = ends[e];
   if ((t & (kRulerEvery - 1)) == 0) return;
-  const uint2 own = reinterpret_cast<const uint2*>(link)[t];
+  const uint2 own = links_of(link, t);
   Chosen c;
   if (!choose_at(uint32_t(t), own, rinfo, chain_info, directed, &c)) return;
   const UnitigPlace pl = place_at_head[c.head_state >> 1];
@@ -2716,7 +2727,7 @@
 constexpr int kLongBlocks = 128;
 
 template <typename KeyT, int kRun, bool kLongPass>
-__device__ __forceinline__ void emit_logged(const DevSet<KeyT>& set, const uint32_t* __restrict__ link,
+__device__ __forceinline__ void emit_logged(const DevSet<KeyT>& set, Links link,
                                             const WalkLog& log, int64_t w, uint64_t hdr, uint32_t u,
                                             uint64_t x_u, const Chosen& c, const UnitigPlace& pl,
                                             uint8_t* __restrict__ bytes) {
@@ -2746,7 +2757,7 @@
     uint32_t cur = u, step = 0;
     int since = 0;
     while (step < steps) {
-      const uint32_t lk = leave_link(link_pair(link, cur), cur);
+      const uint32_t lk = leave_at(link, cur);
       if (lk == kNone) return;
       cur = step_to(cur, lk);
       step++;
@@ -2759,7 +2770,7 @@
 }
 
 template <typename KeyT, int kRun, bool kLongPass>
-__device__ __forceinline__ void emit_ruler_walker(const DevSet<KeyT>& set, const uint32_t* __restrict__ link,
+__device__ __forceinline__ void emit_ruler_walker(const DevSet<KeyT>& set, Links link,
                                                   const unsigned long long* __restrict__ rinfo,
                                                   const WalkLog& log, bool directed, int64_t i, uint64_t x_t,
                                                   const UnitigPlace* __restrict__ place_at_head,
@@ -2786,7 +2797,7 @@
 }
 
 template <typename KeyT, int kRun, bool kLongPass>
-__device__ __forceinline__ void emit_head_walker(const DevSet<KeyT>& set, const uint32_t* __restrict__ link,
+__device__ __forceinline__ void emit_head_walker(const DevSet<KeyT>& set, Links link,
                                                  const unsigned long long* __restrict__ rinfo,
                                                  const unsigned long long* __restrict__ chain_info,
                                                  const WalkLog& log, bool directed, const uint32_t* __restrict__ ends,
@@ -2795,7 +2806,7 @@
   const uint64_t hdr = log.hdr[e];
   if (hdr == kRecUnset) return;
   const uint32_t t = ends[e];
-  const uint2 own = reinterpret_cast<const uint2*>(link)[t];
+  const uint2 own = links_of(link, t);
   Chosen c;
   if (!choose_at(t, own, rinfo, chain_info, directed, &c)) return;
   const uint32_t u = (own.y == kNone && own.x != kNone) ? 2 * t + 1 : 2 * t;
@@ -2804,7 +2815,7 @@
 }
 
 template <typename KeyT, int kRun>
-__global__ __launch_bounds__(256) void k_emit_log_rulers(DevSet<KeyT> set, const uint32_t* __restrict__ link,
+__global__ __launch_bounds__(256) void k_emit_log_rulers(DevSet<KeyT> set, Links link,
                                                           const unsigned long long* __restrict__ rinfo,
                                                           const unsigned long long* __restrict__ chain_info,
                                                           WalkLog log, WalkLog log_heads, bool directed,
@@ -2835,7 +2846,7 @@
 }
 
 template <typename KeyT, int kRun>
-__global__ __launch_bounds__(256) void k_emit_log_heads(DevSet<KeyT> set, const uint32_t* __restrict__ link,
+__global__ __launch_bounds__(256) void k_emit_log_heads(DevSet<KeyT> set, Links link,
                                                          const unsigned long long* __restrict__ rinfo,
                                                          const unsigned long long* __restrict__ chain_info,
                                                          WalkLog log, bool directed,
@@ -2895,7 +2906,7 @@
   int mode = 0;
   ksh_geom g{};
   ksh_set_view set{};
-  uint32_t *nbr = nullptr, *link = nullptr, *head = nullptr, *pos = nullptr, *hlen = nullptr,
+  uint32_t *link0 = nullptr, *link1 = nullptr, *head = nullptr, *pos = nullptr, *hlen = nullptr,
            *hlast = nullptr, *uid = nullptr;
   unsigned long long* info = nullptr;
   uint8_t *ori = nullptr, *hcls = nullptr;
@@ -3004,7 +3015,7 @@
   const int64_t nb = n_buckets(g);
   const int fine_bits = enc_fine_bits(g, n);
   const size_t fine_entries = fine_bits >= 2 ? (size_t(nb) << fine_bits) + 1 : 0;
-  return 2 * al(size_t(2 * n) * 4) + al(size_t(2 * n) * 8) + 5 * al(size_t(n) * 4) + 2 * al(size_t(n)) +
+  return al(size_t(2 * n) * 8) + 7 * al(size_t(n) * 4) + 2 * al(size_t(n)) +
          2 * al(size_t(n) * 8) + al(fine_entries * 4) + al(size_t((n >> kCoarseShift) + 2) * 4) +
          al(sizeof(EncCtl) + size_t(2 * nb) * 4) + 4096;
 }
@@ -3109,8 +3120,8 @@
   KSH_TRY(encode_reserve(ctx, g, n));
   arena_reset(ctx);
   char* at = ctx->slot[kSlotEncode];
-  p->nbr = carve<uint32_t>(at, size_t(2 * n));
-  p->link = carve<uint32_t>(at, size_t(2 * n));
+  p->link0 = carve<uint32_t>(at, size_t(n));
+  p->link1 = carve<uint32_t>(at, size_t(n));
   p->info = carve<unsigned long long>(at, size_t(2 * n));
   p->head = carve<uint32_t>(at, size_t(n));
   p->pos = carve<uint32_t>(at, size_t(n));
@@ -3147,7 +3158,7 @@
     Timer timer(ctx, 3, n);
     const int nbits = g->n_bucket_bits;
     if (directed) {
-      hipLaunchKernelGGL((k_adjacency<KeyT, true>), dim3(nblk(n)), dim3(256), 0, st, set, p->nbr, self_rc_flag);
+      hipLaunchKernelGGL((k_adjacency<KeyT, true>), dim3(nblk(n)), dim3(256), 0, st, set, p->link0, p->link1, self_rc_flag);
     } else if (staged_adjacency() && nbits <= 14 && 2 * g->k >= nbits + 4 &&
                key_bits(g) >= nbits + 2 + (nbits & 1) &&
                n / nb <= 4 * ((kRcWindowBytes - 4 * kRcSegs) / int64_t(sizeof(KeyT) + 6))) {
@@ -3172,8 +3183,8 @@
       int64_t* goff = static_cast<int64_t*>(arena_alloc(ctx, size_t(ng + 1) * 8));
       if (!hist || !totals || !goff) return fail(KSH_INTERNAL, "scratch arena too small");
       RcRecord<KeyT>* rec = reinterpret_cast<RcRecord<KeyT>*>(p->info);
-      uint32_t* rc0 = p->link;
-      uint32_t* rc1 = p->link + n;
+      uint32_t* rc0 = p->link0;
+      uint32_t* rc1 = p->link1;
       const size_t hist_lds = size_t(ng) * 4;
       {
         const uint32_t bit = 1u << (sizeof(KeyT) == 2 ? 0 : sizeof(KeyT) == 4 ? 1 : 2);
@@ -3208,11 +3219,10 @@
       KSH_TRY(scan_exclusive_i64(ctx, totals, goff, ng, goff + ng));
       p->routes |= KSH_ROUTE_PROBE_STAGED | (two_level ? KSH_ROUTE_SCATTER_TWO_LEVEL : 0);
       if (two_level) {
-        RcRecord<KeyT>* tmp_rec = sizeof(RcRecord<KeyT>) == 8 ? rec + n : reinterpret_cast<RcRecord<KeyT>*>(p->nbr);
+        RcRecord<KeyT>* tmp_rec = sizeof(RcRecord<KeyT>) == 8 ? rec + n : reinterpret_cast<RcRecord<KeyT>*>(p->c01);
         uint16_t* tmp_g = reinterpret_cast<uint16_t*>(p->head);
         KSH_BOUND(sizeof(RcRecord<KeyT>) == 8 ? size_t(2 * n) * sizeof(RcRecord<KeyT>) <= al(size_t(2 * n) * 8)
-                                    : reinterpret_cast<char*>(p->link) == reinterpret_cast<char*>(p->nbr) + al(size_t(2 * n) * 4) &&
-                                          size_t(n) * sizeof(RcRecord<KeyT>) <= 2 * al(size_t(2 * n) * 4));
+                                              : size_t(n) * sizeof(RcRecord<KeyT>) <= al(size_t(2 * n) * 8));
         KSH_BOUND(gbits - kSgBits <= 8);
         uint32_t* cursor = rc_cursor;
         constexpr int kPer = sizeof(RcRecord<KeyT>) == 8 ? 4 : 2;
@@ -3274,7 +3284,7 @@
         return !e ? 0 : (std::string(e) == "probe" ? 1 : (std::string(e) == "staged" ? 2 : 0));
       }();
       if (fwd_mode == 1) {
-        hipLaunchKernelGGL((k_adj_fwd<KeyT>), dim3(nblk(n)), dim3(256), 0, st, set, rc0, rc1, p->nbr, self_rc_flag);
+        hipLaunchKernelGGL((k_adj_fwd<KeyT>), dim3(nblk(n)), dim3(256), 0, st, set, rc0, rc1, self_rc_flag);
       } else if (fwd_mode == 0) {
         p->routes |= KSH_ROUTE_FWD_TARGETS;
         constexpr int kTgtChunk = TgtCfg<KeyT>::kChunk, kTgtStreamMax = TgtCfg<KeyT>::kStreamMax;
@@ -3293,7 +3303,7 @@
         hipLaunchKernelGGL((k_tgt_subcuts<KeyT>), dim3(nblk(cap * 8)), dim3(256), 0, st, set, cuts, n_chunks, cap, task,
                            &ctl->tgt_extra, rec);
         hipLaunchKernelGGL((k_adj_fwd_targets<KeyT>), dim3(unsigned(n_chunks + cap)), dim3(kTgtThreads), 0, st, set, rec,
-                           n_chunks, &ctl->tgt_extra, rc0, rc1, p->nbr, self_rc_flag);
+                           n_chunks, &ctl->tgt_extra, rc0, rc1, self_rc_flag);
       } else {
         p->routes |= KSH_ROUTE_FWD_STAGED;
         const int64_t n_chunks = (n + kFwdChunk - 1) / kFwdChunk;
@@ -3301,7 +3311,7 @@
         KSH_BOUND(size_t(n_chunks + 1) * kFwdBounds * 8 <= al(size_t(2 * n) * 8));
         hipLaunchKernelGGL((k_fwd_bounds<KeyT>), dim3(nblk((n_chunks + 1) * 10)), dim3(256), 0, st, set, n_chunks, bounds);
         hipLaunchKernelGGL((k_adj_fwd_staged<KeyT>), dim3(unsigned(n_chunks)), dim3(kFwdChunk), 0, st, set, bounds,
-                           rc0, rc1, p->nbr, self_rc_flag);
+                           rc0, rc1, self_rc_flag);
 #ifdef KSH_FWD_DEBUG
         {
           unsigned long long h[8];
@@ -3315,14 +3325,14 @@
 #endif
       }
     } else {
-      hipLaunchKernelGGL((k_adjacency<KeyT, false>), dim3(nblk(n)), dim3(256), 0, st, set, p->nbr, self_rc_flag);
+      hipLaunchKernelGGL((k_adjacency<KeyT, false>), dim3(nblk(n)), dim3(256), 0, st, set, p->link0, p->link1, self_rc_flag);
     }
   }
   if (directed)
-    hipLaunchKernelGGL((k_link_cut<KeyT, true>), dim3(nblk(n)), dim3(256), 0, st, set, p->nbr);
+    hipLaunchKernelGGL((k_link_cut<KeyT, true>), dim3(nblk(n)), dim3(256), 0, st, set, p->link0, p->link1);
   else
-    hipLaunchKernelGGL((k_link_cut<KeyT, false>), dim3(nblk(n)), dim3(256), 0, st, set, p->nbr);
-  const uint32_t* link = p->nbr;
+    hipLaunchKernelGGL((k_link_cut<KeyT, false>), dim3(nblk(n)), dim3(256), 0, st, set, p->link0, p->link1);
+  const Links link{p->link0, p->link1};
   const int64_t n_hblocks = (n + kHeadSpan - 1) / kHeadSpan;
   int64_t* b01 = p->c23;
   int64_t* b23 = p->c23 + n_hblocks;
@@ -3554,8 +3564,8 @@
   const size_t need = size_t(p->n_bases) + 64;
   uint8_t* bytes;
   void* tmp = nullptr;
-  if (need <= size_t(2 * n) * 4) {
-    bytes = reinterpret_cast<uint8_t*>(p->link);
+  if (need <= size_t(2 * n) * 4 && p->hlast == p->hlen + al(size_t(n) * 4) / 4) {
+    bytes = reinterpret_cast<uint8_t*>(p->hlen);
   } else {
     KSH_TRY(pool_alloc(ctx, need, &tmp));
     bytes = static_cast<uint8_t*>(tmp);
@@ -3563,6 +3573,7 @@
   {
     Timer timer(ctx, 5, n);
     const UnitigPlace* place = reinterpret_cast<const UnitigPlace*>(p->c01);
+    const Links link{p->link0, p->link1};
     const int64_t n_sampled = (n + kRulerEvery - 1) / kRulerEvery;
 #define KSH_EMIT(W, R)                                                                                         \
   do {                                                                                                         \
@@ -3571,15 +3582,15 @@
                          place, bytes);                                                                        \
     } else if (p->log_rulers.hdr) {                                                                            \
       hipLaunchKernelGGL((k_emit_log_rulers<KeyT, R>), dim3(kLongBlocks + nblk(p->log_rulers.n_walkers)),      \
-                         dim3(256), 0, st, set, p->nbr, p->rinfo, p->chain_info, p->log_rulers, p->log_heads,  \
+                         dim3(256), 0, st, set, link, p->rinfo, p->chain_info, p->log_rulers, p->log_heads,    \
                          p->directed, p->ends, place, bytes);                                                  \
       hipLaunchKernelGGL((k_emit_log_heads<KeyT, R>), dim3(nblk(p->log_heads.n_walkers)), dim3(256), 0, st,    \
-                         set, p->nbr, p->rinfo, p->chain_info, p->log_heads, p->directed, p->ends, place,      \
+                         set, link, p->rinfo, p->chain_info, p->log_heads, p->directed, p->ends, place,        \
                          bytes);                                                                               \
     } else {                                                                                                   \
-      hipLaunchKernelGGL((k_emit_rulers<KeyT, R>), dim3(nblk(n_sampled)), dim3(256), 0, st, set, p->nbr,       \
+      hipLaunchKernelGGL((k_emit_rulers<KeyT, R>), dim3(nblk(n_sampled)), dim3(256), 0, st, set, link,         \
                          p->rinfo, p->chain_info, p->directed, place, bytes);                                  \
-      hipLaunchKernelGGL((k_emit_heads<KeyT, R>), dim3(nblk(p->n_ends)), dim3(256), 0, st, set, p->nbr,        \
+      hipLaunchKernelGGL((k_emit_heads<KeyT, R>), dim3(nblk(p->n_ends)), dim3(256), 0, st, set, link,          \
                          p->rinfo, p->chain_info, p->directed, p->ends, p->n_ends, place, bytes);              \
     }                                                                                                          \
   } while (0)
```

New measurement: 28270 (median of 2 runs). About the same (+0.3%).
